# Xinglab/abPOA

Measured on AMD Instinct MI355X. Metric: read-sets/sec (consensus bit-exact) + DP Gcells/sec (roofline.dp_gcells_per_s), higher is better.
Workload: dtype int16

## Files before the change

### abpoa_amd/csrc/backtrack_dir.h

```cpp
#pragma once
#include "dp_common.h"
#include "dir_plane.h"
#include "rows_fast.h"
#include "backtrack.h"

namespace abpoa_hip {

constexpr int DBTR = 256;
constexpr int DIR_TRI_SLACK = 9;
constexpr int DIR_NA = -32768;
template <int R> struct __attribute__((aligned(16))) DirBtT { int2 rec[R]; int2 pd[R]; int32_t stg[R], rowA[R]; };
typedef DirBtT<DBTR> DirBt;

constexpr int SPEC_PM_ROWS = 256;
constexpr int SPEC_WK = 4;
__device__ __forceinline__ bool dir_walk_pair(const DevBatch &b, const AlnDesc &d) { return d.n_rows >= 768 && d.cigar_cap < 65536 && d.qlen < 65536 && b.ret_cigar; }
template <typename T, int GAP, int DBR = DBTR>
__device__ __forceinline__ void finish_alignment_dir(const DevBatch &b, const AlnDesc &d, AlnOut *out_rec, const TailState &ts, const int role = -1,
                                                     int *spec_ctl = nullptr, const int gen = 0) {
    constexpr int PN = Width<T>::PN, CW = FastFmt<T, GAP>::CW, DB = DirFmt<T, GAP>::DB, S = (int)sizeof(T);
    constexpr int ALIGN = 16 / DB;
    constexpr int DBL = DB == 2 ? 1 : 2;
    constexpr int NQ = DBR / 64;
    typedef DirBtT<DBR> DirBt;
    typedef typename std::conditional<GAP == 1, uint16_t, uint32_t>::type DW;
    typedef __attribute__((address_space(3))) unsigned char lds_byte_t;
    typedef __attribute__((address_space(3))) DW lds_dw_t;
    typedef int v2i_t __attribute__((ext_vector_type(2)));
    typedef __attribute__((address_space(3))) v2i_t lds_i2_t;
    typedef __attribute__((address_space(3))) int lds_i32_t;
    const int lane = threadIdx.x & 63;
    const int gn = d.n_rows, qlen = d.qlen;
    const int o1 = b.o1, o2 = b.o2;
    GLOBAL_AS const uint8_t *row_base = vgpr_ptr(b.row_base + d.row0);
    GLOBAL_AS const int32_t *row_node_id = vgpr_ptr(b.row_node_id + d.row0);
    GLOBAL_AS const uint32_t *row_pd = vgpr_ptr(b.row_pd + 2 * d.row0);
    GLOBAL_AS const int32_t *pred_off = vgpr_ptr(b.pred_off + d.poff0), *pred_row = vgpr_ptr(b.pred_row + d.pred0);
    GLOBAL_AS int32_t *g_bsn = vgpr_ptr(b.dp_beg_sn + d.row0), *g_esn = vgpr_ptr(b.dp_end_sn + d.row0);
    GLOBAL_AS int64_t *g_coff = vgpr_ptr(b.row_cell_off + d.row0);
    T *planes = (T *)(b.planes + d.plane_off);
    const unsigned char *arena = (const unsigned char *)planes;
    int status = ts.status, best_score = ts.best_score, best_i = ts.best_i, best_j = ts.best_j, bt_steps = 0;
    WG_SYNC();
    typedef __attribute__((address_space(3))) volatile int lds_vint_t;
    const bool spec_static = role >= 0 && dir_walk_pair(b, d), spec = spec_static && status == 0;
    auto start_row = [&](int r_) __attribute__((always_inline)) { return (int)(((long long)gn * (SPEC_WK - r_)) / SPEC_WK); };
    const int R_g = spec && role >= 1 ? start_row(role) : 0, R_lo = R_g - SPEC_PM_ROWS + 1;
    const int total_lds = b.lds.bt_off + b.lds.bt_bytes_tail;
    const int half_lds = spec_static ? ((total_lds - (SPEC_WK - 1) * SPEC_PM_ROWS * 4) / SPEC_WK) & ~15 : total_lds;
    int *pm_all = (int *)(lds_raw + b.lds.phase_off + SPEC_WK * half_lds);
    int *pm = pm_all + (role >= 1 ? role - 1 : 0) * SPEC_PM_ROWS;
    lds_vint_t *ctl = (lds_vint_t *)spec_ctl, *my = ctl + 8 * (role > 0 ? role : 0);
    auto helper_out = [&](int st_) __attribute__((always_inline)) { if (lane == 0) my[1] = st_; asm volatile("s_waitcnt lgkmcnt(0)" ::: "memory"); if (lane == 0) my[0] = gen; };
    if (role >= 1) {
        if (!spec) { if (spec_static) helper_out(-1); return; }
        const int c_g = __builtin_amdgcn_readfirstlane(gld_i32(vgpr_ptr(b.row_max_i + d.row0) + R_g));
        if (c_g < 1 || c_g > qlen) { helper_out(-1); return; }
        best_i = R_g; best_j = c_g;
    }

    const int cwr = takes_wide(b, d) ? (sizeof(T) == 2 ? (GAP == 2 ? 4 : 2) : 2) : CW;
    if (status == 0 && role < 1) {
        const int k0 = __builtin_amdgcn_readfirstlane(pred_off[gn - 1]), k1 = __builtin_amdgcn_readfirstlane(pred_off[gn]);
        for (int kb = k0; kb < k1; kb += 64) {
            const int k = kb + lane; const bool v = k < k1;
            int in_row = 0, end = 0, score = INT_MIN;
            if (v) {
                in_row = pred_row[k];
                const int pe = g_esn[in_row], pb = g_bsn[in_row];
                const int dpe = (pe + 1) * PN - 1; end = qlen > dpe ? dpe : qlen;
                score = (int)planes[g_coff[in_row] - (long long)(pe - pb + 1) * cwr * PN + (long long)(end - pb * PN) * cwr];
            }
            const int mx = wave_max_i32(score);
            if (mx > best_score) {
                const int first = __builtin_ctzll(__ballot(v && score == mx));
                best_score = mx; best_i = __builtin_amdgcn_readlane(in_row, first); best_j = __builtin_amdgcn_readlane(end, first);
            }
        }
    }

    int n_cigar = 0, node_s = 0, node_e = 0, query_s = 0, query_e = 0, n_aln = 0, n_match = 0;
    long long win_ticks = 0, walk_ticks = 0; int n_windows = 0, n_general = 0;
    long long dbg_why = 0, dbg_a = 0, dbg_b = 0;
    if (spec_static && role == 0) {
        for (int t = lane; t < (SPEC_WK - 1) * SPEC_PM_ROWS; t += 64) pm_all[t] = 0;
        asm volatile("s_waitcnt lgkmcnt(0)" ::: "memory");
        if (lane == 0) ctl[0] = gen;
    }
    if (status == 0 && b.ret_cigar && d.cigar_cap < gn + qlen + 2) status = ABPOA_HIP_EBACKTRACK;
    if (role >= 1 && status != 0) { helper_out(-1); return; }
    if (status == 0 && b.ret_cigar) {
        const int lds0 = b.lds.phase_off + (role >= 1 ? role * half_lds : 0);
        DirBt &B = *(DirBt *)(lds_raw + lds0);
        unsigned char *win = lds_raw + lds0 + (int)sizeof(DirBt);
        const int win_bytes = half_lds - (int)sizeof(DirBt);
        GLOBAL_AS uint64_t *cg = vgpr_ptr(b.cigar + d.cigar_off + (role >= 1 ? (long long)role * d.cigar_cap : 0));
        bool merged = false; int idx1 = 0, met = 0;
        int t_next = (role > 0 ? role : 0) + 1;
        int w_lo = 1, w_hi = 0, w_cref = 0; bool w_tri = false;
        unsigned nx_end = 0; bool nx_ok = false;
        auto load_window = [&](int hi, int jtop) __attribute__((always_inline)) -> int {
            const long long tw0 = (long long)__builtin_amdgcn_s_memtime(); ++n_windows;
            WG_SYNC();
            bool early = nx_ok && hi == w_lo - 1;
            const unsigned e_lo = nx_end > (unsigned)win_bytes ? nx_end - (unsigned)win_bytes : 0u;
            if (early) {
                const int n16 = (int)((nx_end - e_lo) >> 4);
                const int4 *src = (const int4 *)(arena + e_lo); int4 *dst = (int4 *)win;
                for (int i0 = 0; i0 < n16; i0 += 64) {
                    const int idx = i0 + lane;
                    if (idx < n16) __builtin_amdgcn_global_load_lds((const __attribute__((address_space(1))) void *)(src + idx), (__attribute__((address_space(3))) void *)(dst + i0), 16, 0, 0);
                }
            }
            const int cref = jtop - 4096;
            int bs[NQ], es[NQ]; long long co[NQ]; unsigned pdv[NQ], pdh[NQ];
#pragma unroll
            for (int q = 0; q < NQ; ++q) {
                const int r = hi - 64 * q - lane, rc = imax(r, 1);
                bs[q] = g_bsn[rc]; es[q] = g_esn[rc]; co[q] = g_coff[rc]; pdv[q] = row_pd[2 * rc]; pdh[q] = row_pd[2 * rc + 1];
            }
            int W[NQ], pc[NQ]; unsigned sa[NQ]; bool vq[NQ];
#pragma unroll
            for (int q = 0; q < NQ; ++q) { vq[q] = hi - 64 * q - lane >= 1; W[q] = (es[q] - bs[q] + 1) * PN; pc[q] = bs[q] * PN; sa[q] = (unsigned)(co[q] * S); }
            const unsigned end_hi = (unsigned)__builtin_amdgcn_readfirstlane((int)(sa[0] + (unsigned)(W[0] * DB)));
            int r_full = 0;
#pragma unroll
            for (int q = 0; q < NQ; ++q) r_full += __builtin_popcountll(__ballot(vq[q] && (early ? sa[q] >= e_lo : end_hi - sa[q] <= (unsigned)win_bytes)));
            if (early && r_full == 0) {
                asm volatile("s_waitcnt vmcnt(0)" ::: "memory");
                early = false; nx_ok = false;
#pragma unroll
                for (int q = 0; q < NQ; ++q) r_full += __builtin_popcountll(__ballot(vq[q] && end_hi - sa[q] <= (unsigned)win_bytes));
            }
            const bool narrow = early || r_full >= imin(16, hi);
            int sl[NQ], ns[NQ], off[NQ], R;
            unsigned s_lo = 0;
            if (narrow) {
                R = r_full;
                const int ql = (R - 1) >> 6, ll = (R - 1) & 63;
#pragma unroll
                for (int q = 0; q < NQ; ++q) if (q == ql) s_lo = (unsigned)__builtin_amdgcn_readlane((int)sa[q], ll);
                nx_end = s_lo;
                if (early) s_lo = e_lo;
#pragma unroll
                for (int q = 0; q < NQ; ++q) { sl[q] = pc[q]; ns[q] = W[q]; off[q] = (int)(sa[q] - s_lo); }
            } else {
                int run = 0; R = 0;
#pragma unroll
                for (int q = 0; q < NQ; ++q) {
                    const int tl = imax(pc[q], (jtop - 64 * q - lane - DIR_TRI_SLACK) & ~(ALIGN - 1)), th = imin(pc[q] + W[q], (jtop + ALIGN) & ~(ALIGN - 1));
                    sl[q] = tl; ns[q] = vq[q] ? imax(0, th - tl) : 0;
                    const int incl = run + wave_scan_add_i32(ns[q] * DB);
                    off[q] = incl - ns[q] * DB; run = __builtin_amdgcn_readlane(incl, 63);
                    R += __builtin_popcountll(__ballot(vq[q] && incl <= win_bytes));
                }
                if (R < 1) R = 1;
            }
            const int lo = hi - R + 1;
            nx_ok = narrow;
            if (narrow && early) {}
            else if (narrow) {
                const int n16 = (int)((end_hi - s_lo) >> 4);
                const int4 *src = (const int4 *)(arena + s_lo); int4 *dst = (int4 *)win;
                for (int i0 = 0; i0 < n16; i0 += 64) {
                    const int idx = i0 + lane;
                    if (idx < n16) __builtin_amdgcn_global_load_lds((const __attribute__((address_space(1))) void *)(src + idx), (__attribute__((address_space(3))) void *)(dst + i0), 16, 0, 0);
                }
            } else {
#pragma unroll
                for (int q = 0; q < NQ; ++q) {
                    const unsigned srcq = sa[q] + (unsigned)((sl[q] - pc[q]) * DB);
                    const int nrow = imin(64, R - 64 * q);
                    for (int u = 0; u < nrow; ++u) {
                        const int n_ = __builtin_amdgcn_readlane(ns[q], u) * DB / 16, ob = __builtin_amdgcn_readlane(off[q], u);
                        const unsigned so = (unsigned)__builtin_amdgcn_readlane((int)srcq, u);
                        const int4 *sp = (const int4 *)(arena + so); unsigned char *dp = win + ob;
                        for (int i0 = 0; i0 < n_; i0 += 64)
                            if (i0 + lane < n_) __builtin_amdgcn_global_load_lds((const __attribute__((address_space(1))) void *)(sp + i0 + lane),
                                    (__attribute__((address_space(3))) void *)(dp + i0 * 16), 16, 0, 0);
                    }
                }
            }
            int A[NQ];
#pragma unroll
            for (int q = 0; q < NQ; ++q) {
                A[q] = off[q] - ((sl[q] - cref) << DBL);
                const int li = hi - 64 * q - lane - lo;
                if (vq[q] && li >= 0) { B.rowA[li] = A[q]; B.pd[li] = make_int2((int)pdv[q], (int)pdh[q]); B.stg[li] = (sl[q] & 0x7fff) | ((sl[q] > pc[q] ? 1 : 0) << 15) | (ns[q] << 16); }
            }
            WG_SYNC();
#pragma unroll
            for (int q = 0; q < NQ; ++q) {
                const int r = hi - 64 * q - lane, li = r - lo;
                if (!(vq[q] && li >= 0)) continue;
                int pk[2];
#pragma unroll
                for (int k = 0; k < 2; ++k) {
                    const int dk = (int)((pdv[q] >> (8 * k)) & 0xffu), pr = r - dk; const bool in = dk != 255 && pr >= lo;
                    pk[k] = in ? (dk | (((B.rowA[pr - lo] >> 1) & 0xffff) << 8)) : 255;
                }
                B.rec[li] = make_int2(pk[0], pk[1]);
            }
            asm volatile("s_waitcnt vmcnt(0)" ::: "memory");
            WG_SYNC();
            w_lo = lo; w_hi = hi; w_cref = cref;
            win_ticks += (long long)__builtin_amdgcn_s_memtime() - tw0;
            w_tri = !narrow;
            return __builtin_amdgcn_readfirstlane(A[0]);
        };
        uint64_t last_word = 0; bool have_pending = false;
        auto store_word = [&](int idx, uint64_t wv) __attribute__((always_inline)) {
            GLOBAL_AS uint64_t *p_ = cg + idx;
            const int lo_ = (int)(wv & 0xffffffffull), hi_ = (int)(wv >> 32);
            asm volatile("global_store_dwordx2 %0, %1, off" :: "v"(p_), "v"(make_int2(lo_, hi_)) : "memory");
        };
        auto push = [&](int op, int len, int node_row, int query_id) __attribute__((always_inline)) {
            const uint64_t L = (uint64_t)(int64_t)len;
            if (n_cigar == 0 || op != ABPOA_HIP_CINS || op != (int)(last_word & 0xf)) {
                if (have_pending) store_word(n_cigar - 1, last_word);
                const uint64_t n_id = (uint64_t)(int64_t)node_row, q_id = (uint64_t)(int64_t)query_id;
                if (op == ABPOA_HIP_CMATCH) last_word = n_id << 34 | q_id << 4 | (uint64_t)op;
                else if (op == ABPOA_HIP_CINS) last_word = q_id << 34 | L << 4 | (uint64_t)op;
                else last_word = n_id << 34 | L << 4 | (uint64_t)op;
                have_pending = true; ++n_cigar;
            } else last_word += L << 4;
        };
        int runv = 0, run_n = 0, run_j = 0;
        auto flush_run = [&]() __attribute__((always_inline)) {
            if (run_n == 0) return;
            if (have_pending) { store_word(n_cigar - 1, last_word); have_pending = false; }
            if (spec) {
                const int row_ = lane < run_n ? runv : -1, col_ = run_j - lane;
                const int row_first = __builtin_amdgcn_readlane(runv, 0);
                while (t_next < SPEC_WK && row_first < start_row(t_next) - SPEC_PM_ROWS + 1) ++t_next;
                if (t_next < SPEC_WK) {
                    const int tl_ = row_ - (start_row(t_next) - SPEC_PM_ROWS + 1);
                    const bool in2 = row_ >= 0 && (unsigned)tl_ < (unsigned)SPEC_PM_ROWS;
                    const int e_ = in2 ? ((lds_vint_t *)(pm_all + (t_next - 1) * SPEC_PM_ROWS))[tl_] : 0;
                    const unsigned long long hit_ = __ballot(in2 && e_ != 0 && (e_ & 0xffff) == col_);
                    if (hit_) { const int f_ = __builtin_ctzll(hit_); idx1 = (int)((unsigned)__builtin_amdgcn_readlane(e_, f_) >> 16); met = t_next; run_n = f_; merged = true; if (run_n == 0) return;
                            }
                }
                if (role >= 1) { const int t_ = row_ - R_lo; if (lane < run_n && (unsigned)t_ < (unsigned)SPEC_PM_ROWS) pm[t_] = col_ | ((n_cigar + lane) << 16); }
            }
            if (lane < run_n) cg[n_cigar + lane] = (uint64_t)(unsigned)runv << 34 | (uint64_t)(unsigned)(run_j - 1 - lane) << 4 | (uint64_t)ABPOA_HIP_CMATCH;
// ... 210 lines not shown
```

### abpoa_amd/csrc/engine.cpp

```cpp
#include <hip/hip_runtime.h>
#include <stdio.h>
#include <stdlib.h>
#include <string.h>
#include <stdarg.h>
#include <limits.h>
#include <mutex>
#include <vector>
#include <algorithm>
#include "engine_options.h"
#include "batch_stream.h"
#include "dir_plane.h"

namespace abpoa_hip {

static char g_err[512] = ""; static std::mutex g_err_mu;
static thread_local char g_err_copy[512] = "";
static thread_local char tl_err[512] = "";
void set_err(const char *fmt, ...) {
    va_list ap; va_start(ap, fmt); vsnprintf(tl_err, sizeof(tl_err), fmt, ap); va_end(ap);
    std::lock_guard<std::mutex> lk(g_err_mu);
    memcpy(g_err, tl_err, sizeof(g_err));
}
const char *thread_last_error() { return tl_err; }
void clear_thread_error() { tl_err[0] = 0; }
#define HIP_TRY(expr, code)                                                                          \
    do { hipError_t e_ = (expr); if (e_ != hipSuccess) {                                             \
        set_err("%s failed: %s (%s:%d)", #expr, hipGetErrorString(e_), __FILE__, __LINE__); return code; } } while (0)

int Blob::reserve(size_t n) {
    if (n <= cap) return 0;
    size_t want = std::max(n, cap + cap / 2);
    want = (want + 0xFFFFF) & ~(size_t)0xFFFFF;
    release();
    if (hipMalloc((void **)&dev, want) != hipSuccess) { dev = nullptr; set_err("hipMalloc(%zu) failed", want); return ABPOA_HIP_ENOMEM; }
    if (mirrored && hipHostMalloc((void **)&host, want, hipHostMallocDefault) != hipSuccess) {
        host = nullptr; set_err("hipHostMalloc(%zu) failed", want); return ABPOA_HIP_ENOMEM; }
    cap = want; return 0;
}
void Blob::release() { if (dev) (void)hipFree(dev); if (host) (void)hipHostFree(host); dev = host = nullptr; cap = 0; }

struct Engine {
    bool ready = false; int device = -1;
    BatchStream flat;
    abpoa_hip_stats_t stats{};
    std::mutex mu, stats_mu;
};
static Engine g;
long long g_dbg[10] = {0};
long long g_dir_counts[2] = {0, 0};

int engine_device() { return g.ready ? g.device : -1; }
void add_global_stats(const StreamStats &s) {
    std::lock_guard<std::mutex> lk(g.stats_mu);
    g.stats.n_launches += s.n_launches; g.stats.n_alignments += s.n_alignments; g.stats.n_cells += s.n_cells;
    g.stats.algo_bytes += s.algo_bytes; g.stats.kernel_ms += s.kernel_ms; g.stats.h2d_ms += s.h2d_ms; g.stats.d2h_ms += s.d2h_ms; g.stats.tail_ms += s.tail_ms; g.stats.rounds_ms += s.rounds_ms;
    g.stats.rounds_launches += s.rounds_launches; g.stats.rounds_algo_bytes += s.rounds_algo_bytes;
}

static size_t align_up(size_t x, size_t a = 256) { return (x + a - 1) / a * a; }

int BatchStream::open(int device) {
    if (open_) return 0;
    HIP_TRY(hipSetDevice(device), ABPOA_HIP_ENODEV);
    HIP_TRY(hipStreamCreateWithFlags(&stream_, hipStreamNonBlocking), ABPOA_HIP_ENODEV);
    for (auto &e : ev_) HIP_TRY(hipEventCreate(&e), ABPOA_HIP_ENODEV);
    device_ = device; open_ = true; return 0;
}
void BatchStream::close() {
    if (!open_) return;
    (void)hipSetDevice(device_);
    (void)hipStreamSynchronize(stream_);
    in_.release(); out_.release(); planes_.release();
    for (auto &e : ev_) (void)hipEventDestroy(e);
    (void)hipStreamDestroy(stream_);
    open_ = false;
}

#ifdef ABPOA_HIP_WIDE_W3
constexpr int WIDE_PER_CU_MAX = 12, WIDE_RING_MIN = 2;
#else
constexpr int WIDE_PER_CU_MAX = 8, WIDE_RING_MIN = 4;
#endif
void make_lds_plan(const abpoa_hip_scoring_t *sc, int max_qlen, int max_bits, int64_t est_cols, int n_aln, LdsPlan *Lp) {
    LdsPlan &L = *Lp;
    const int P = sc->gap_mode == ABPOA_HIP_LINEAR_GAP ? 1 : (sc->gap_mode == ABPOA_HIP_AFFINE_GAP ? 3 : 5);
    const int cell = max_bits / 8, npr = P == 1 ? 1 : (P == 3 ? 2 : 3);
    const bool longq = max_qlen + 1 > 16384;
    L.q_off = 0; L.q_cap = max_qlen + 1 <= 32000 ? (int)align_up(max_qlen + 1, 16) : 0;
    L.mat_off = L.q_cap; L.mx_off = L.mat_off + (int)align_up(4 * sc->m * sc->m, 16);
    L.phase_off = L.mx_off + (int)align_up(4 * sc->m * (sc->m + 1), 16);
    L.ring_off = lds_fixed_bytes_dp(); L.ring_rows = 16; L.ring_cols = (int)align_up((size_t)est_cols, 64);
    while ((int64_t)L.ring_rows * npr * L.ring_cols * cell > 40 * 1024 && L.ring_rows > 4) L.ring_rows /= 2;
    if ((int64_t)L.ring_rows * npr * L.ring_cols * cell > 40 * 1024) L.ring_cols = 0;
    const int ring_bytes = L.ring_rows * npr * L.ring_cols * cell;
    L.bt_off = lds_fixed_bytes_bt();
    L.bt_bytes = std::max(std::max(8 * 1024, std::min(24 * 1024, (longq ? 62 : 38) * 1024 - L.phase_off - L.bt_off)), L.ring_off + ring_bytes - L.bt_off) & ~15;
    const int fw = P == 1 ? 1 : (max_bits == 16 ? (P == 3 ? 1 : 2) : (P == 3 ? 2 : 3));
    L.fr_off = 0; L.fr_rows = 16; L.fr_cols = fw ? std::max(128, (int)align_up((size_t)est_cols, 64)) : 0;
    const int fr_budget = (longq ? 62 : 36) * 1024 - L.phase_off;
    while (L.fr_cols && (int64_t)L.fr_rows * fw * (L.fr_cols + 4) * 4 + 64 > fr_budget && L.fr_rows > 4) L.fr_rows /= 2;
    if (L.fr_cols && (int64_t)L.fr_rows * fw * (L.fr_cols + 4) * 4 + 64 > fr_budget) L.fr_cols = 0;
    if (L.q_cap == 0 || est_cols > 1024) L.fr_cols = 0;
    { const char *nf_ = opt_env("ABPOA_HIP_NOFAST"); if (nf_ && atoi(nf_)) L.fr_cols = 0; }
    const int fr_bytes = L.fr_cols ? L.fr_rows * fw * (L.fr_cols + 4) * 4 + 64 : 0;
    L.total = L.phase_off + std::max(std::max(L.ring_off + ring_bytes, L.bt_off + L.bt_bytes), L.fr_off + fr_bytes);
    L.bt_bytes_tail = std::max(8 * 1024, std::min(28 * 1024, (longq ? 62 : 38) * 1024 - L.phase_off - L.bt_off)) & ~15;
    { const int per_cu = std::max(1, (n_aln + 255) / 256);
      if (per_cu < 4 && L.fr_cols > 128) L.bt_bytes_tail = std::max(L.bt_bytes_tail, std::min(56 * 1024, 160 * 1024 / per_cu - 2048 - L.phase_off - L.bt_off) & ~15); }
    if (n_aln > 4 * 256 && L.fr_cols && L.fr_cols <= 128) L.bt_bytes_tail = std::min(L.bt_bytes_tail, 12 * 1024);
    { const char *tb_ = opt_env("ABPOA_HIP_BT_BYTES"); if (tb_ && atoi(tb_) >= 4096 && atoi(tb_) <= 65536) L.bt_bytes_tail = atoi(tb_) & ~15; }
    L.total_rows = L.phase_off + L.fr_off + fr_bytes; L.total_tail = L.phase_off + L.bt_off + L.bt_bytes_tail;
    L.bt_wc = 0; { const char *wc_ = opt_env("ABPOA_HIP_BT_WC"); if (wc_ && atoi(wc_) >= 8 && atoi(wc_) <= 64) L.bt_wc = atoi(wc_) & ~7; }
    L.loc_rows = L.loc_cols = L.total_local = 0;
    if (sc->align_mode == ABPOA_HIP_LOCAL_MODE && sc->wb < 0 && P != 1 && L.q_cap && !(opt_env("ABPOA_HIP_NOFAST") && atoi(opt_env("ABPOA_HIP_NOFAST")))) {
        const int lw = P == 3 ? 1 : 2;
        L.loc_cols = 9 * 64; L.loc_rows = 16;
        while ((int64_t)L.loc_rows * lw * (L.loc_cols + 4) * 4 > 60 * 1024 - L.phase_off && L.loc_rows > 4) L.loc_rows /= 2;
        L.total_local = L.phase_off + L.fr_off + (int)align_up((size_t)L.loc_rows * lw * (L.loc_cols + 4) * 4, 16) + 256;
    }
    L.wide_nw = 0; L.wfr_rows = L.wfr_cols = L.wx_off = L.total_wide = 0; L.wide_w_lo = 1; L.wide_w_hi = 0; L.narrow_off = 0; L.w_mx_off = L.w_phase_off = 0;
    { const char *nw_ = opt_env("ABPOA_HIP_NOWIDE"), *mw_ = opt_env("ABPOA_HIP_TEAM");
      if (L.fr_cols && L.q_cap && !(nw_ && atoi(nw_))) {
          L.wide_nw = 1;
          if (mw_ && (atoi(mw_) == 1 || atoi(mw_) == 2 || atoi(mw_) == 4)) L.wide_nw = atoi(mw_);
          L.wfr_cols = (est_cols > WIDE_RING_COLS && !(opt_env("ABPOA_HIP_NOXL") && atoi(opt_env("ABPOA_HIP_NOXL")))) ? WIDE_RING_COLS_XL : WIDE_RING_COLS; L.wfr_rows = 16;
          if (sc->m > 16) L.wide_nw = 0;
          L.w_mx_off = (int)align_up((size_t)(max_qlen + 2) / 2, 16); L.w_phase_off = L.w_mx_off + (int)align_up(4 * sc->m * (sc->m + 1), 16);
          const int fww = (P == 5 && max_bits == 32) ? 2 : fw;
          if (P == 5 && (sc->gap_open1 + sc->gap_ext1 >= 65535 || sc->gap_open2 + sc->gap_ext2 >= 65535)) L.wide_nw = 0;
          L.wide_w_lo = 40; L.wide_w_hi = (L.wfr_cols - 2 * 8 - 1) / 2;
          { const char *lo_ = opt_env("ABPOA_HIP_WIDE_LO"); if (lo_ && atoi(lo_) > 0) L.wide_w_lo = atoi(lo_); }
          const char *rr_env_ = opt_env("ABPOA_HIP_RING_ROWS");
          if (rr_env_ && atoi(rr_env_) >= 4) L.wfr_rows = atoi(rr_env_) >= 16 ? 16 : (atoi(rr_env_) >= 8 ? 8 : 4); else rr_env_ = nullptr;
          const int budget = 120 * 1024 - L.w_phase_off - 512;
          while ((int64_t)L.wfr_rows * fww * (L.wfr_cols + 4) * 4 > budget && L.wfr_rows > 4) L.wfr_rows /= 2;
          const int extra_ = L.wide_nw > 1 ? 16 * 16 + 64 : 0;
          auto per_cu_ = [&](int rows_) { return std::min<int64_t>(WIDE_PER_CU_MAX, 128 / ((L.w_phase_off + (int64_t)rows_ * fww * (L.wfr_cols + 4) * 4 + extra_ + 1279) / 1280)); };
          if (!(rr_env_)) {
              const int top_ = L.wfr_rows; int best_ = top_;
              for (int r_ = top_; r_ >= WIDE_RING_MIN; r_ /= 2) {
                  if (per_cu_(r_) > per_cu_(best_)) best_ = r_;
                  if (per_cu_(r_) * 256 >= std::min(n_aln, WIDE_PER_CU_MAX * 256)) { best_ = r_; break; }
              }
              L.wfr_rows = best_;
          }
          L.wx_off = L.fr_off + (int)align_up((size_t)L.wfr_rows * fww * (L.wfr_cols + 4) * 4, 16);
          L.total_wide = L.w_phase_off + L.wx_off + extra_;
          if (P == 1) L.wide_nw = 0;
      } }
}

int BatchStream::prepare(const abpoa_hip_scoring_t *sc, int n, const BatchShape *sh, unsigned flags) {
    if (!open_) { set_err("stream not open"); return ABPOA_HIP_ENODEV; }
    HIP_TRY(hipSetDevice(device_), ABPOA_HIP_ENODEV);
    sc_ = *sc; mat_.assign(sc->mat, sc->mat + sc->m * sc->m); sc_.mat = mat_.data();
    flags_ = flags; n_ = n;
    P_ = sc->gap_mode == ABPOA_HIP_LINEAR_GAP ? 1 : (sc->gap_mode == ABPOA_HIP_AFFINE_GAP ? 3 : 5);
    const bool banded = sc->wb >= 0;
    desc_.resize(n); recs_.resize(n); full_cells_.resize(n); est_cells_.resize(n); dir_full_cells_.resize(n); dir_est_cells_.resize(n); trace_arena_.clear();
    rows_tot_ = preds_tot_ = outs_tot_ = q_tot_ = cig_tot_ = 0;
    for (int i = 0; i < n; ++i) {
        AlnDesc &d = desc_[i];
        d.n_rows = sh[i].n_rows; d.qlen = sh[i].qlen;
        d.bits = abpoa_hip_score_bits(sc, d.n_rows, d.qlen, &d.inf_min);
        d.w = sc->wb < 0 ? d.qlen : sc->wb + (int)(sc->wf * d.qlen);
        d.cigar_cap = d.n_rows + d.qlen + 8;
        d.query_off = q_tot_; d.row0 = rows_tot_; d.poff0 = rows_tot_ + i; d.pred0 = preds_tot_; d.out0 = outs_tot_; d.cigar_off = cig_tot_;
        q_tot_ += d.qlen; rows_tot_ += d.n_rows; preds_tot_ += sh[i].n_pred; outs_tot_ += sh[i].n_out; cig_tot_ += d.cigar_cap;
        const int pn = d.bits == 16 ? 16 : 8;
        const int64_t width = (int64_t)((d.qlen + pn) / pn) * pn;
        const int pv = sc->gap_mode == ABPOA_HIP_LINEAR_GAP ? 2 : (sc->gap_mode == ABPOA_HIP_AFFINE_GAP ? 4 : 8);
        full_cells_[i] = width * pv * d.n_rows;
        int64_t est = banded ? std::min<int64_t>(width, 2LL * d.w + 3 * pn + 32) : width;
        { const char *pct_ = opt_env("ABPOA_HIP_ARENA_PCT"); if (pct_ && atoi(pct_) > 0 && atoi(pct_) < 100) est = std::max<int64_t>(pn, est * atoi(pct_) / 100); }
        d.plane_cap = std::min<int64_t>(full_cells_[i], width * pv + est * pv * (d.n_rows - 1));
        est_cells_[i] = d.plane_cap;
        const int64_t dbc = (sc->gap_mode == ABPOA_HIP_AFFINE_GAP ? 2 : 4) * 8 / d.bits + 1;
        dir_full_cells_[i] = width * (pv + dbc) * d.n_rows + 64;
        dir_est_cells_[i] = std::min<int64_t>(dir_full_cells_[i], width * (pv + dbc) + (est * dbc + est * pv / 4 + 2 * pn) * (d.n_rows - 1));
    }
    size_t o = 0;
    auto take = [&](size_t bytes) { size_t at = o; o = align_up(o + bytes); return at; };
    o_desc_ = take(sizeof(AlnDesc) * n); o_mat_ = take(sizeof(int32_t) * sc->m * sc->m); o_query_ = take(q_tot_ + 1);
    o_base_ = take(rows_tot_); o_sdist_ = take(rows_tot_); o_pd_ = take(8 * rows_tot_); o_nid_ = take(4 * rows_tot_); o_rem_ = take(4 * rows_tot_); o_act_ = take(rows_tot_);
    o_poff_ = take(4 * (rows_tot_ + n)); o_pred_ = take(4 * (preds_tot_ + 1)); o_ooff_ = take(4 * (rows_tot_ + n)); o_out_ = take(4 * (outs_tot_ + 1) + 4 * 512);
    in_bytes_ = o;
    o = 0;
    o_rec_ = take(sizeof(AlnOut) * n); o_cig_ = take(8 * cig_tot_); o_left_ = take(4 * rows_tot_); o_right_ = take(4 * rows_tot_);
    o_bsn_ = take(4 * rows_tot_); o_esn_ = take(4 * rows_tot_); o_coff_ = take(8 * rows_tot_); o_rmi_ = take(4 * rows_tot_);
    out_bytes_ = o;
    int rc;
    if ((rc = in_.reserve(in_bytes_)) || (rc = out_.reserve(out_bytes_))) return rc;
    memcpy(in_.host + o_mat_, sc->mat, sizeof(int32_t) * sc->m * sc->m);
    memset(in_.host + o_act_, 1, rows_tot_);
    return 0;
}

ProblemSlots BatchStream::slots(int i) const {
    const AlnDesc &d = desc_[i]; uint8_t *hi = in_.host, *ho = out_.host; ProblemSlots s;
    s.query = hi + o_query_ + d.query_off; s.row_base = hi + o_base_ + d.row0;
    s.row_node_id = (int32_t *)(hi + o_nid_) + d.row0; s.row_remain = (int32_t *)(hi + o_rem_) + d.row0; s.row_active = hi + o_act_ + d.row0;
    s.pred_off = (int32_t *)(hi + o_poff_) + d.poff0; s.pred_row = (int32_t *)(hi + o_pred_) + d.pred0;
    s.out_off = (int32_t *)(hi + o_ooff_) + d.poff0; s.out_row = (int32_t *)(hi + o_out_) + d.out0;
    s.left = (int32_t *)(ho + o_left_) + d.row0; s.right = (int32_t *)(ho + o_right_) + d.row0;
    return s;
}
const uint64_t *BatchStream::cigar(int i) const { return (const uint64_t *)(out_.host + o_cig_) + desc_[i].cigar_off; }
const int32_t *BatchStream::left(int i) const { return (const int32_t *)(out_.host + o_left_) + desc_[i].row0; }
const int32_t *BatchStream::right(int i) const { return (const int32_t *)(out_.host + o_right_) + desc_[i].row0; }

int BatchStream::run() {
    HIP_TRY(hipSetDevice(device_), ABPOA_HIP_ENODEV);
    const abpoa_hip_scoring_t *sc = &sc_;
    const bool banded = sc->wb >= 0, trace = flags_ & BS_TRACE, fresh = flags_ & BS_FRESH_BAND;
    const int P = P_, n = n_;
    uint8_t *hi = in_.host, *ho = out_.host, *di = in_.dev, *dout = out_.dev;
    std::vector<int> todo(n); for (int i = 0; i < n; ++i) todo[i] = i;
    const size_t lr_words = (o_right_ - o_left_) / 4 + rows_tot_;
    std::vector<int32_t> saved_lr;
    bool first_pass = true; int rc;
    std::vector<AlnDesc> pass;
    const bool dirtrace = trace && opt_env("ABPOA_HIP_DIRTRACE") && atoi(opt_env("ABPOA_HIP_DIRTRACE"));
    bool dir = (!trace || dirtrace) && banded && sc->align_mode == ABPOA_HIP_GLOBAL_MODE && dir_plane_usable(sc->gap_mode, sc->gap_open1, sc->gap_ext1, sc->gap_open2, sc->gap_ext2) &&
               !(opt_env("ABPOA_HIP_NODIR") && atoi(opt_env("ABPOA_HIP_NODIR"))) && !(opt_env("ABPOA_HIP_TEAM") && atoi(opt_env("ABPOA_HIP_TEAM")) > 1);
    for (int i = 0; i < n; ++i) {
        AlnDesc &d = desc_[i]; bool ok = banded || (sc->align_mode == ABPOA_HIP_LOCAL_MODE && sc->wb < 0);
        if (ok && memchr(hi + o_act_ + d.row0, 0, (size_t)d.n_rows)) ok = false;
        if (ok && banded && !fresh) {
            const int32_t *l = (const int32_t *)(ho + o_left_) + d.row0, *r = (const int32_t *)(ho + o_right_) + d.row0;
            for (int k = 0; k < d.n_rows && ok; ++k) ok = l[k] == d.n_rows && r[k] == 0;
        }
        d.flags = ok ? ALN_FAST_OK : 0; d.pad0 = 0;
    }
    if (dir) {
        for (int i = 0; i < n; ++i) {
            AlnDesc &d = desc_[i];
            if (!(d.flags & ALN_FAST_OK)) continue;
            const int32_t *po = (const int32_t *)(hi + o_poff_) + d.poff0, *pr = (const int32_t *)(hi + o_pred_) + d.pred0; uint8_t *sd = hi + o_sdist_ + d.row0;
            uint32_t *pdw = (uint32_t *)(hi + o_pd_) + 2 * d.row0;
            memset(sd, 0, (size_t)d.n_rows);
            bool ok = true;
            for (int r = 0; r < d.n_rows && ok; ++r) {
                const int np_ = po[r + 1] - po[r];
                if (np_ > DIR_K_MAX && r < d.n_rows - 1) ok = false;
                uint64_t pdv = ~0ull;
                for (int k = po[r]; k < po[r + 1]; ++k) {
                    const int p_ = pr[k], dist = r == d.n_rows - 1 ? 255 : std::min(255, r - p_); if (dist > sd[p_]) sd[p_] = (uint8_t)dist;
                    const int t = k - po[r]; if (t < 8 && r - p_ <= 254) pdv = (pdv & ~(0xffull << (8 * t))) | ((uint64_t)(r - p_) << (8 * t));
                }
                (void)np_;
                pdw[2 * r] = (uint32_t)pdv; pdw[2 * r + 1] = (uint32_t)(pdv >> 32);
            }
            if (!ok) d.flags = 0;
        }
    }
    while (!todo.empty()) {
        int64_t plane_bytes = 0;
        pass.resize(todo.size());
        for (size_t t = 0; t < todo.size(); ++t) pass[t] = desc_[todo[t]];
        DevBatch b; memset(&b, 0, sizeof(b));
        b.n = (int)pass.size(); b.m = sc->m;
        {
            int max_qlen = 0, max_bits = 16; int64_t est_cols = 0;
            for (const AlnDesc &d : pass) {
// ... 302 lines not shown
```

### abpoa_amd/csrc/engine.h

```cpp
#pragma once
#include <stdint.h>
#include <hip/hip_runtime.h>
#include "../../include/abpoa_hip.h"

namespace abpoa_hip {

struct AlnDesc {
    int32_t n_rows, qlen;
    int32_t bits;
    int32_t inf_min;
    int32_t w;
    int32_t cigar_cap;
    int32_t flags;
    int32_t pad0;
    int64_t query_off;
    int64_t row0;
    int64_t poff0;
    int64_t pred0;
    int64_t out0;
    int64_t plane_off;
    int64_t plane_cap;
    int64_t cigar_off;
};

struct AlnOut {
    int32_t status;
    int32_t best_score, best_row, best_col;
    int32_t node_s, node_e, query_s, query_e;
    int32_t n_aln_bases, n_matched_bases;
    int32_t n_cigar;
    int32_t pad;
    int64_t n_cells;
    int64_t cells_used;
    int64_t clk_dp, clk_bt;
    int32_t n_rows_done, n_bt_steps;
    int64_t seg[6];
};

#define ALN_FAST_OK 1
#define ALN_SKIP 2
#define WIDE_RING_COLS 448
#define WIDE_RING_COLS_XL 704
#define ABPOA_HIP_STATUS_OVERFLOW 1
#define ABPOA_HIP_STATUS_NEED_SCORES 2

struct LdsPlan {
    int32_t q_off, q_cap;
    int32_t mat_off;
    int32_t phase_off;
    int32_t ring_rows, ring_cols;
    int32_t ring_off;
    int32_t bt_off, bt_bytes;
    int32_t bt_bytes_tail;
    int32_t bt_wc;
    int32_t fr_off, fr_rows, fr_cols;
    int32_t wfr_rows, wfr_cols, wx_off, wide_nw;
    int32_t wide_w_lo, wide_w_hi;
    int32_t narrow_off;
    int32_t total_wide;
    int32_t w_mx_off, w_phase_off;
    int32_t loc_rows, loc_cols, total_local;
    int32_t mx_off;
    int32_t total;
    int32_t total_rows, total_tail;
};

struct DevBatch {
    int32_t n;
    int32_t m;
    int32_t o1, e1, o2, e2;
    int32_t align_mode, gap_mode, wb, zdrop, ret_cigar, rev_cigar;
    int32_t want_trace;
    int32_t dbg;
    int32_t fresh_band;
    int32_t want_lr;
    int32_t bits_mask;
    int32_t dir_mode;
    int32_t pad1;
    LdsPlan lds;
    const int32_t *mat;
    const AlnDesc *aln;
    AlnOut *out;
    const uint8_t *query;
    const uint8_t *row_base;
    const int32_t *row_node_id;
    const int32_t *row_remain;
    const uint8_t *row_active;
    const uint8_t *row_sdist;
    const uint32_t *row_pd;
    const int32_t *pred_off;
    const int32_t *pred_row;
    const int32_t *out_off;
    const int32_t *out_row;
    int32_t *left, *right;
    int32_t *dp_beg_sn, *dp_end_sn;
    int64_t *row_cell_off;
    int32_t *row_max_i;
    uint8_t *planes;
    uint64_t *cigar;
};

constexpr int LINEAR_FAST_W = 40;
__host__ __device__ inline bool fast_global_job(int gap_mode, int align_mode, int wb, int e1) {
    if (wb < 0) return false;
    if (gap_mode == ABPOA_HIP_LINEAR_GAP && e1 < 1) return false;
    return align_mode == ABPOA_HIP_GLOBAL_MODE || align_mode == ABPOA_HIP_EXTEND_MODE;
}
__host__ __device__ inline bool fast_global_aln(int gap_mode, int w, int pad0) { return gap_mode != ABPOA_HIP_LINEAR_GAP || w + (pad0 >> 1) < LINEAR_FAST_W; }

int lds_fixed_bytes_dp();
int lds_fixed_bytes_bt();

hipError_t launch_dp(const DevBatch &b, int n_fast, hipStream_t stream, hipEvent_t after_rows);
hipError_t launch_dp_fast(const DevBatch &b, hipStream_t stream, hipEvent_t after_rows);
hipError_t launch_dp_general(const DevBatch &b, hipStream_t stream);

}
```

### abpoa_amd/csrc/engine_options.cpp

```cpp
#include "engine_options.h"
#include <atomic>
#include <cstdlib>
#include <cstring>
#include <mutex>
#include <string>

namespace abpoa_hip {
namespace {

struct Row { const char *name, *help; };
const Row kTable[] = {
    {"ABPOA_GPU_DEVICES", "P  device ordinals abpoa_hip_msa_batch spreads its batches over: all | 0,1,... (default: the device of abpoa_hip_init)"},
    {"ABPOA_GPU_BATCHES_PER_DEVICE", "P  batches dealt per device queue [2]"},
    {"ABPOA_HIP_STRICT", "P  1: a call that would hand any read-set to the host driver fails with ABPOA_HIP_ESTRICT"},
    {"ABPOA_HIP_VERBOSE", "P  per-pass timings, residency and fallback reasons on stderr"},
    {"ABPOA_HIP_HOSTGRAPH", "T  1: the host driver for every job"},
    {"ABPOA_HIP_NO_DEVICE_STRAND", "T  1: -s jobs on the host driver"},
    {"ABPOA_HIP_NO_DEVICE_LOCAL", "T  1: local-mode jobs on the host driver"},
    {"ABPOA_HIP_NO_DEVICE_GENERAL", "T  1: general-kernel jobs on the host driver"},
    {"ABPOA_HIP_DEVICE_GENERAL", "T  1: the general kernel for every device-resident job"},
    {"ABPOA_HIP_LOCKSTEP", "T  1: one launch per phase and round also where the all-rounds kernel would run"},
    {"ABPOA_HIP_NODIR", "T  1: score-record arenas instead of direction words"},
    {"ABPOA_HIP_DIR_WIDE", "T  1 / 0: direction words for wide-band alignments always / never (default: by residency and memory)"},
    {"ABPOA_HIP_NOFAST", "T  1: no fast row loops (general kernel)"},
    {"ABPOA_HIP_NOWIDE", "T  1: no wide row loop"},
    {"ABPOA_HIP_NOXL", "T  1: no long-read form of the wide row loop"},
    {"ABPOA_HIP_TEAM", "T  1 | 2 | 4 wavefronts per wide-band alignment"},
    {"ABPOA_HIP_LOCAL_TEAM", "T  1 / 0: the four-wavefront local row loop always / never"},
    {"ABPOA_HIP_WIDE_LO", "T  smallest band half-width that takes the wide loop [40]"},
    {"ABPOA_HIP_RING_ROWS", "T  depth of the wide loop's score ring (4 | 8 | 16)"},
    {"ABPOA_HIP_EXTRA_ROUTE_MIN", "T  ragged sets with fewer extra columns keep the narrow loop"},
    {"ABPOA_HIP_NO_RAGGED_SPLIT", "T  1: read-sets with ragged read ends stay in the batch of the uniform ones (no all-rounds kernel for such a job)"},
    {"ABPOA_HIP_RAGGED_CONCURRENT", "T  1: the ragged batch of a mixed job runs on a second queue of the device beside the uniform batch (measured: see LOG.md)"},
    {"ABPOA_HIP_PASS_SETS", "T  read-sets per pass of the device-resident driver"},
    {"ABPOA_HIP_FIRST_PASS", "T  start the node-slot ladder at pass 1 / 2 / 3 (profiling runs of one step)"},
    {"ABPOA_HIP_NO_PASS_HINT", "T  1: always start the ladder at 3x"},
    {"ABPOA_HIP_GROUPS", "T  read-set groups of the host driver"},
    {"ABPOA_HIP_ARENA_PCT", "T  arena estimate in percent (overflow-retry tests)"},
    {"ABPOA_HIP_BT_BYTES", "T  LDS window of the tail kernel in bytes"},
    {"ABPOA_HIP_BT_WC", "T  columns per row of the tail's column-slice windows"},
    {"ABPOA_HIP_ORDER_LDS", "T  0: the row-order walk with global tables"},
    {"ABPOA_HIP_ORDER_CAP", "T  node capacity of the row-order walk's LDS tables"},
    {"ABPOA_HIP_DBG", "D  bit mask handed to the kernels (DevBatch.dbg: 64 no fast loops, 128 keep counters, 1024 one wavefront per backtrack, 2048 the compiler's tight loop, ...)"},
    {"ABPOA_HIP_DEVSYNC", "D  1: compare device graph / row order / MSA with the host's after every read"},
    {"ABPOA_HIP_DEVICE_AUDIT", "D  1: every pool of a device queue must sit on that queue's device"},
    {"ABPOA_HIP_CIGAR_DIGEST", "D  1: fold every graph cigar into a per-set digest on the device"},
    {"ABPOA_HIP_DIRTRACE", "D  1: keep direction words and scores (word-level tests)"},
    {"ABPOA_HIP_IMBAL", "D  1: per-round mean / slowest alignment"},
    {"ABPOA_HIP_WIDE_COUNTERS", "D  path census of the wide loop (diagnostic build)"},
    {"ABPOA_HIP_ROW_CENSUS", "D  row census of the narrow loop (diagnostic build)"},
    {"ABPOA_HIP_ORDER_PROF", "D  in-kernel clock of the row-order walk (diagnostic build)"},
};
constexpr int N = (int)(sizeof(kTable) / sizeof(kTable[0]));

struct Snap { bool set[N]; std::string val[N]; };
std::mutex g_mu;
bool g_over_on[N]; std::string g_over[N];
std::atomic<const Snap *> g_snap{nullptr};

int find(const char *name) { for (int i = 0; i < N; ++i) if (strcmp(kTable[i].name, name) == 0) return i; return -1; }

}

void refresh_options() {
    std::lock_guard<std::mutex> lk(g_mu);
    Snap s;
    for (int i = 0; i < N; ++i) {
        const char *e = g_over_on[i] ? g_over[i].c_str() : getenv(kTable[i].name);
        s.set[i] = e != nullptr; s.val[i] = e ? e : "";
    }
    const Snap *cur = g_snap.load(std::memory_order_acquire);
    bool same = cur != nullptr;
    for (int i = 0; same && i < N; ++i) same = cur->set[i] == s.set[i] && cur->val[i] == s.val[i];
    if (!same) g_snap.store(new Snap(s), std::memory_order_release);
}

const char *opt_env(const char *name) {
    const Snap *cur = g_snap.load(std::memory_order_acquire);
    if (!cur) { refresh_options(); cur = g_snap.load(std::memory_order_acquire); }
    const int i = find(name);
    return (i >= 0 && cur->set[i]) ? cur->val[i].c_str() : nullptr;
}

int set_option(const char *name, const char *value) {
    const int i = name ? find(name) : -1;
    if (i < 0) return -1;
    { std::lock_guard<std::mutex> lk(g_mu); g_over_on[i] = value != nullptr; g_over[i] = value ? value : ""; }
    refresh_options();
    return 0;
}

int list_options(const char **names, const char **help, int cap) {
    for (int i = 0; i < N && i < cap; ++i) { if (names) names[i] = kTable[i].name; if (help) help[i] = kTable[i].help; }
    return N;
}

}
```

### abpoa_amd/csrc/fast_tail.h

```cpp
#pragma once
#include "rows_fast.h"
#include "rows_local.h"
#include "backtrack.h"
#include "backtrack_dir.h"

namespace abpoa_hip {

template <typename T, int GAP, bool DIR = false>
__device__ __forceinline__ void align_fast_tail(const DevBatch &b, const AlnDesc &d, AlnOut *out_rec, const int role = -1, int *spec_ctl = nullptr, const int gen = 0) {
    const int lane = threadIdx.x & 63;
    if (role >= 1) {
        if (!(DIR && takes_dir(b, d) && dir_walk_pair(b, d))) return;
        typedef __attribute__((address_space(3))) volatile int lds_vint_t;
        while (((lds_vint_t *)spec_ctl)[0] != gen) __builtin_amdgcn_s_sleep(4);
    }
    uint8_t *s_query = lds_raw + b.lds.q_off;
    int32_t *s_mat = (int32_t *)(lds_raw + b.lds.mat_off);
    const bool dir_a = DIR && takes_dir(b, d);
    if (!dir_a) { GLOBAL_AS const int32_t *g_mat = vgpr_ptr(b.mat); for (int i = lane; i < b.m * b.m; i += 64) s_mat[i] = g_mat[i]; }
    if (!dir_a) { GLOBAL_AS const uint8_t *g_query = vgpr_ptr(b.query + d.query_off); for (int i = lane; i < d.qlen; i += 64) s_query[i] = g_query[i]; }
    TailState ts;
    ts.status = out_rec->status; ts.n_cells = out_rec->n_cells; ts.cursor = out_rec->cells_used; ts.rows_done = out_rec->n_rows_done;
    ts.best_score = d.inf_min; ts.best_i = 0; ts.best_j = 0;
    if (b.align_mode == ABPOA_HIP_LOCAL_MODE || b.align_mode == ABPOA_HIP_EXTEND_MODE) { ts.best_score = out_rec->best_score; ts.best_i = out_rec->best_row; ts.best_j = out_rec->best_col; }
    for (int i_ = 0; i_ < 6; ++i_) ts.seg[i_] = out_rec->seg[i_];
    ts.clk1 = (long long)__builtin_amdgcn_s_memtime(); ts.clk0 = ts.clk1 - out_rec->clk_dp;
    WG_SYNC();
    if constexpr (DIR) {
        if (!takes_dir(b, d)) finish_alignment<T, GAP, FastFmt<T, GAP>::CW>(b, d, out_rec, ts);
        else if (role >= 0 && dir_walk_pair(b, d)) finish_alignment_dir<T, GAP, 64>(b, d, out_rec, ts, role, spec_ctl, gen);
        else if (role <= 0) finish_alignment_dir<T, GAP>(b, d, out_rec, ts);
    }
    else finish_alignment<T, GAP, FastFmt<T, GAP>::CW>(b, d, out_rec, ts);
}

}
```

### abpoa_amd/csrc/msa_device.cpp

```cpp
#include <algorithm>
#include <atomic>
#include <chrono>
#include <limits.h>
#include <mutex>
#include <stdio.h>
#include <stdlib.h>
#include <string.h>
#include <thread>
#include <vector>
#include <hip/hip_runtime.h>
#include "engine_options.h"
#include "batch_stream.h"
#include "msa_device.h"
#include "poa_device.h"
#include "poa_graph.h"
#include "dir_plane.h"
#include "msa_batch.h"
#include "msa_device_debug.h"

namespace abpoa_hip {

namespace {
#define HIP_OK(expr, code) do { hipError_t e_ = (expr); if (e_ != hipSuccess) { \
        set_err("%s failed: %s (%s:%d)", #expr, hipGetErrorString(e_), __FILE__, __LINE__); return code; } } while (0)
// ... 82 lines not shown
    const bool fast = fast_global_job(sc->gap_mode, sc->align_mode, sc->wb, sc->gap_ext1) || (sc->gap_mode != ABPOA_HIP_LINEAR_GAP && sc->align_mode == ABPOA_HIP_LOCAL_MODE);
    if (!fast && opt_env("ABPOA_HIP_NO_DEVICE_GENERAL") && atoi(opt_env("ABPOA_HIP_NO_DEVICE_GENERAL"))) return false;
    return true;
}

int msa_device_resident_sets(const abpoa_hip_scoring_t *sc, int n_sets, const abpoa_hip_readset_t *sets) {
    int max_qlen = 0; for (int s = 0; s < n_sets; ++s) for (int r = 0; r < sets[s].n_reads; ++r) max_qlen = std::max(max_qlen, sets[s].lens[r]);
    if (max_qlen <= 0) return 0;
    const int w_max = sc->wb + (int)(sc->wf * (float)max_qlen);
    LdsPlan pl; int32_t inf_d; const int mb = abpoa_hip_score_bits(sc, 3 * max_qlen + 1024, max_qlen, &inf_d); const int pn_ = mb == 16 ? 16 : 8;
    make_lds_plan(sc, max_qlen, mb, std::min<int64_t>((int64_t)((max_qlen + pn_) / pn_) * pn_, 2LL * w_max + 3 * pn_ + 32), n_sets, &pl);
    if (pl.wide_nw != 1 || !(w_max >= pl.wide_w_lo && w_max <= pl.wide_w_hi) || pl.total_wide <= 0) return 0;
    int dev = 0, cus = 256; if (hipGetDevice(&dev) == hipSuccess) { hipDeviceProp_t pr;
            if (hipGetDeviceProperties(&pr, dev) == hipSuccess && pr.multiProcessorCount > 0) cus = pr.multiProcessorCount; }
#ifdef ABPOA_HIP_WIDE_W3
    const int per_cu = std::max(1, std::min(12, 128 / ((pl.total_wide + 1279) / 1280)));
#else
    const int per_cu = std::max(1, std::min(8, 128 / ((pl.total_wide + 1279) / 1280)));
#endif
    return per_cu * cus;
}

static int run_msa_device_body(const abpoa_hip_scoring_t *sc_in, int n_sets, const abpoa_hip_readset_t *sets, abpoa_hip_msa_t *out, int n_threads,
                               std::vector<int> *fallback, DeviceRunStats *stats, double node_factor, unsigned flags, int device, int slot, bool force_general, bool *want_general,
                               std::vector<int> *fallback_reason) {
    abpoa_hip_scoring_t sc_norm = *sc_in; const bool local = sc_in->align_mode == ABPOA_HIP_LOCAL_MODE, extend = sc_in->align_mode == ABPOA_HIP_EXTEND_MODE;
    if (local) sc_norm.wb = -1;
    const abpoa_hip_scoring_t *sc = &sc_norm;
    const bool amb = flags & ABPOA_HIP_AMB_STRAND;
    const bool want_msa = flags & ABPOA_HIP_OUT_MSA, want_cons = (flags & ABPOA_HIP_OUT_CONS) || !want_msa;
    if (slot < 0 || slot >= MSA_DEVICE_SLOTS) { set_err("bad device slot %d", slot); return ABPOA_HIP_EINVAL; }
    std::lock_guard<std::mutex> lk(g_cache_mu[slot]);
    Cache &C = g_cache[slot];
    if (device < 0) device = engine_device();
    if (device < 0) { set_err("engine not initialised"); return ABPOA_HIP_ENODEV; }
    HIP_OK(hipSetDevice(device), ABPOA_HIP_ENODEV);
    t_queue_device = device;
    if (C.device != device) {
        if (C.device >= 0) {
            (void)hipSetDevice(C.device);
            for (Arena *a : {&C.in, &C.graph, &C.rows, &C.planes, &C.out, &C.msa}) { if (a->dev) (void)hipFree(a->dev);
                    if (a->host) (void)hipHostFree(a->host); *a = Arena(); }
            if (C.stream) (void)hipStreamDestroy(C.stream); if (C.copy_stream) (void)hipStreamDestroy(C.copy_stream);
            if (C.ev_copy) (void)hipEventDestroy(C.ev_copy);
            for (hipEvent_t e : C.ev) (void)hipEventDestroy(e);
            C = Cache();
            HIP_OK(hipSetDevice(device), ABPOA_HIP_ENODEV);
        }
        if (!C.stream) HIP_OK(hipStreamCreateWithFlags(&C.stream, hipStreamNonBlocking), ABPOA_HIP_ENODEV);
        C.device = device;
    }
    fallback->clear();
    if (stats) memset(stats, 0, sizeof(*stats));
    const double t_begin = now_s();
    const int CW = sc->gap_mode == ABPOA_HIP_LINEAR_GAP ? 2 : (sc->gap_mode == ABPOA_HIP_AFFINE_GAP ? 4 : 8);
    const bool unbanded = sc->wb < 0;
    int max_reads = 0, max_qlen = 0; int64_t tot_reads = 0, tot_bases = 0, max_cap0 = 0;
    for (int s = 0; s < n_sets; ++s) {
        max_reads = std::max(max_reads, sets[s].n_reads); tot_reads += sets[s].n_reads;
        int64_t sum = 0; int mx = 0;
        for (int r = 0; r < sets[s].n_reads; ++r) { max_qlen = std::max(max_qlen, sets[s].lens[r]); mx = std::max(mx, sets[s].lens[r]); sum += sets[s].lens[r];
                }
        tot_bases += sum; max_cap0 = std::max(max_cap0, std::min<int64_t>(2 + sum, 2 + (int64_t)(node_factor * mx) + 1024));
    }
    bool general;
    {   LdsPlan pl; int32_t inf_d; const int mb = abpoa_hip_score_bits(sc, (int)max_cap0, max_qlen, &inf_d); const int pn_ = mb == 16 ? 16 : 8;
        const int64_t width_ = (int64_t)((max_qlen + pn_) / pn_) * pn_, w_ = sc->wb + (int)(sc->wf * (float)max_qlen);
        make_lds_plan(sc, max_qlen, mb, (local || unbanded) ? width_ : std::min<int64_t>(width_, 2LL * w_ + 3 * pn_ + 32), n_sets, &pl);
        bool fast_global = fast_global_job(sc->gap_mode, sc->align_mode, sc->wb, sc->gap_ext1) && pl.fr_cols > 0 && max_qlen <= pl.q_cap;
        if (fast_global && sc->gap_mode == ABPOA_HIP_LINEAR_GAP) {
            if (w_ >= LINEAR_FAST_W) fast_global = false;
            for (int s = 0; s < n_sets && fast_global; ++s) if (msa_device_set_is_ragged(sets[s])) fast_global = false;
        }
        const bool fast_local = local && sc->gap_mode != ABPOA_HIP_LINEAR_GAP && mb == 16 && pl.loc_cols > 0 && (max_qlen / 16 + 1) * 16 <= pl.loc_cols
                && max_qlen <= pl.q_cap;
        general = !(fast_global || fast_local);
        if (opt_env("ABPOA_HIP_DEVICE_GENERAL") && atoi(opt_env("ABPOA_HIP_DEVICE_GENERAL"))) general = true;
        if (force_general) general = true;
    }
    const bool roomy = node_factor >= 4096.0;
    const int in_cap = roomy ? std::max((int)POA_IN_CAP, std::min(250, max_reads + 1)) : POA_IN_CAP, out_cap = roomy ? std::max((int)POA_OUT_CAP, std::min(250, max_reads + 1)) : POA_OUT_CAP;
    const bool dir = !local && !extend && !general && !amb && in_cap <= POA_IN_CAP && dir_plane_usable(sc->gap_mode, sc->gap_open1, sc->gap_ext1, sc->gap_open2,
            sc->gap_ext2) && !(opt_env("ABPOA_HIP_NODIR") && atoi(opt_env("ABPOA_HIP_NODIR"))) &&
                     !(opt_env("ABPOA_HIP_TEAM") && atoi(opt_env("ABPOA_HIP_TEAM")) > 1);
    const int DB = sc->gap_mode == ABPOA_HIP_AFFINE_GAP ? 2 : 4;

    std::vector<PoaSet> ps(n_sets);
    int64_t node_tot = 0, pred_tot = 0, cig_tot = 0, scr_tot = 0, plane_tot = 0, read_i = 0, cons_tot = 0, term_tot = 0; int max_node_cap = 0;
    const int w_max = sc->wb + (int)(sc->wf * (float)max_qlen);
    const int aln_cap = std::max(1, sc->m - 1), rid_words = want_msa ? std::max(1, (max_reads + 63) / 64) : 0;
    auto est_cols = [&](int64_t width, int w, int pn) { return (local || unbanded) ? width : std::min<int64_t>(width, 2LL * w + 3 * pn + 32); };
    int wide_lo = 1, wide_hi = 0, wide_ring_rows = 16;
    { LdsPlan pl; int32_t inf_d; const int mb = abpoa_hip_score_bits(sc, 3 * max_qlen + 1024, max_qlen, &inf_d); const int pn_ = mb == 16 ? 16 : 8;
      make_lds_plan(sc, max_qlen, mb, est_cols((int64_t)((max_qlen + pn_) / pn_) * pn_, w_max, pn_), n_sets, &pl);
      if (pl.wide_nw >= 1 && !local && !general) { wide_lo = pl.wide_w_lo; wide_hi = pl.wide_w_hi; wide_ring_rows = pl.wfr_rows; } }
    std::vector<int> extra(n_sets, 0), route(n_sets, 0); int max_extra = 0, weff_lo = INT_MAX, weff_hi = 0;
    const int route_min = opt_env("ABPOA_HIP_EXTRA_ROUTE_MIN") ? atoi(opt_env("ABPOA_HIP_EXTRA_ROUTE_MIN")) : 0;
    if (!local && !general && sc->wb >= 0) for (int s = 0; s < n_sets; ++s) {
        int mx = 0, mn = INT_MAX; for (int r = 0; r < sets[s].n_reads; ++r) { mx = std::max(mx, sets[s].lens[r]); mn = std::min(mn, sets[s].lens[r]); }
        if (sets[s].n_reads < 2) continue;
        const int spread = mx - mn, tol = std::max(64, mx / 8);
        extra[s] = spread > tol ? std::min((spread + 15) & ~15, 2048) : 0;
        max_extra = std::max(max_extra, extra[s]);
        route[s] = extra[s] >= route_min ? extra[s] : 0;
        weff_lo = std::min(weff_lo, sc->wb + (int)(sc->wf * (float)mn) + route[s] / 2);
        weff_hi = std::max(weff_hi, sc->wb + (int)(sc->wf * (float)mx) + route[s] / 2);
    }
    if (weff_hi == 0) { weff_lo = 0; }
    const bool lin_fast = !general && !local && !extend && sc->gap_mode == ABPOA_HIP_LINEAR_GAP && !amb;
    const bool rounds_possible = (dir || lin_fast) && max_reads > 2 && !(w_max >= wide_lo && wide_hi >= wide_lo) && max_extra == 0;
    bool dir_wide = false, any_wide_set = false;
    { const char *e_ = opt_env("ABPOA_HIP_DIR_WIDE"); if (dir && e_ && atoi(e_) > 0) dir_wide = true; }
    const bool dir_wide_auto = dir && !opt_env("ABPOA_HIP_DIR_WIDE");
    if (dir_wide_auto && wide_ring_rows <= 4 && wide_hi >= wide_lo) dir_wide = true;
    for (int s = 0; s < n_sets; ++s) {
        PoaSet &S = ps[s]; memset(&S, 0, sizeof(S));
        int64_t sum = 0; int mx = 0;
        for (int r = 0; r < sets[s].n_reads; ++r) { sum += sets[s].lens[r]; mx = std::max(mx, sets[s].lens[r]); }
        const int64_t cap = std::min<int64_t>(2 + sum, 2 + (int64_t)((node_factor + (extra[s] > 0 ? 1.0 : 0.0)) * mx) + 1024);
        S.n_reads = sets[s].n_reads; S.node_cap = (int)cap; S.pred_cap = (int)(4 * cap);
        S.read0 = read_i; read_i += sets[s].n_reads;
        S.term0 = term_tot; term_tot += sets[s].n_reads + 2;
        S.node0 = node_tot; node_tot += cap + 1;
        S.pred0 = pred_tot; pred_tot += S.pred_cap;
        S.cigar_cap = (int)(cap + mx + 8); S.cigar_off = cig_tot; cig_tot += ((rounds_possible && S.cigar_cap < 65536) ? 4 : 1) * (int64_t)S.cigar_cap;
        S.scratch0 = scr_tot; scr_tot += 3LL * max_qlen + 4 * cap + 8;
        S.cons_cap = (int)std::min<int64_t>(cap, 2LL * mx + 64); S.cons0 = cons_tot; cons_tot += S.cons_cap;
        const int w = sc->wb + (int)(sc->wf * (float)mx) + route[s] / 2;
        S.band_extra = route[s];
        max_node_cap = std::max(max_node_cap, (int)cap);
        any_wide_set |= (w >= wide_lo && w <= wide_hi);
    }
    auto size_arenas = [&](bool dw) {
        plane_tot = 0;
        for (int s = 0; s < n_sets; ++s) {
            PoaSet &S = ps[s]; int mx = 0; for (int r = 0; r < sets[s].n_reads; ++r) mx = std::max(mx, sets[s].lens[r]);
            const int64_t cap = S.node_cap;
            int32_t inf_dummy; const int bits = abpoa_hip_score_bits(sc, (int)cap, mx, &inf_dummy); const int pn = bits == 16 ? 16 : 8;
            const int64_t width = (int64_t)((mx + pn) / pn) * pn;
            const int w = sc->wb + (int)(sc->wf * (float)mx);
            int64_t est = std::min<int64_t>(width, est_cols(width, w, pn) + extra[s]);
            int64_t sum_len = 0; for (int r = 0; r < sets[s].n_reads; ++r) sum_len += sets[s].lens[r];
            const bool slots_fixed = 2 + sum_len <= 2 + (int64_t)(3.0 * mx) + 1024;
            if (node_factor > 3.0 && (roomy || slots_fixed)) {
                const double cellb = dir ? (double)(DB + 8) : (double)CW * (bits / 8);
                int64_t e2 = roomy ? width : std::min<int64_t>(width, (int64_t)((double)est * node_factor / 3.0));
                if (roomy && (double)e2 * (double)cap * cellb > 1e9) e2 = std::min<int64_t>(width, est * 4);
                est = std::max(est, e2);
            }
            const bool wide_s = !local && w + route[s] / 2 >= wide_lo && w + route[s] / 2 <= wide_hi;
            const bool dir_s = dir && (dw || !wide_s);
            const int64_t rec_div = (wide_s && wide_ring_rows <= 4) ? 2 : 4;
            const int64_t recb = wide_s ? ((bits == 16 && CW == 4) ? 4 : 8) : CW * (bits / 8);
            const int64_t bytes = local ? (int64_t)up((size_t)((width * cap + 64) * CW * (bits / 8) + 64 * 8 * 4))
                                : dir_s ? (int64_t)up((size_t)(width * (DB + recb) + (est * DB + est * recb / rec_div + 32) * (cap - 1) + 64 * 8 * 4))
                                      : (int64_t)up((size_t)((width + est * (cap - 1)) * CW * (bits / 8) + 64 * 8 * 4));
            S.plane_off = plane_tot; S.plane_cap = bytes - 64 * 8 * 4; plane_tot += bytes;
        }
    };
    size_arenas(dir_wide);
    Layout L; size_t o = 0;
    auto take = [&](size_t bytes) { size_t at = o; o = up(o + bytes); return at; };
    L.o_sets = take(sizeof(PoaSet) * n_sets); L.o_roff = take(8 * (tot_reads + 1)); L.o_rlen = take(4 * (tot_reads + 1)); L.o_mat = take(4 * sc->m * sc->m);
    L.o_rargs = take(poa_rounds_args_bytes()); L.o_msaoff_h = take(want_msa ? 8 * (size_t)n_sets : 0);
    bool any_w = false; for (int s = 0; s < n_sets && !any_w; ++s) any_w = sets[s].weights != nullptr;
    L.o_wts = take(any_w ? 4 * (size_t)(tot_bases + 64) : 0);
    L.o_reads = take(tot_bases + 64); L.in_bytes = o;
    L.o_rc = take(amb ? tot_bases + 64 : 0); L.o_wrc = take(amb && any_w ? 4 * (size_t)(tot_bases + 64) : 0); L.in_dev_bytes = o;
    o = 0;
    L.o_state = take(sizeof(PoaState) * n_sets);
    L.o_cnode = take(4 * cons_tot); L.o_ccov = take(4 * cons_tot); L.o_cbase = take(cons_tot); L.o_isrc = take(amb ? (size_t)tot_reads : 0);
    const size_t dl_bytes = o;
    L.o_order0 = take(4 * node_tot); L.o_order1 = take(4 * node_tot); L.o_base = take(node_tot); L.o_nout = take(node_tot);
    L.o_out = take(4 * node_tot * POA_HOT); L.o_outw = take(4 * node_tot * POA_HOT); L.o_nread = take(4 * node_tot);
    L.o_outx = take(4 * node_tot * (size_t)(out_cap - POA_HOT)); L.o_outwx = take(4 * node_tot * (size_t)(out_cap - POA_HOT));
    L.o_inx = take(4 * node_tot * (size_t)(in_cap - POA_HOT));
    L.o_nin = take(node_tot); L.o_naln = take(node_tot); L.o_in = take(4 * node_tot * POA_HOT); L.o_aln = take(4 * node_tot * (size_t)aln_cap);
    L.o_row = take(4 * node_tot);
    L.o_rid = take(8 * node_tot * (size_t)out_cap * (size_t)rid_words); L.o_mrank = take(want_msa ? 4 * node_tot : 0);
    L.o_msaoff = take(want_msa ? 8 * (size_t)n_sets : 0);
    L.o_tout = take(4 * term_tot); L.o_toutw = take(4 * term_tot); L.o_tin = take(4 * term_tot);
    L.graph_bytes = o;
    o = 0;
    L.o_ticket = take(4 * POA_CU_TICKETS);
    L.o_aln_desc = take(sizeof(AlnDesc) * n_sets); L.o_out_rec = take(sizeof(AlnOut) * n_sets);
    L.o_rbase = take(node_tot); L.o_rsd = take(node_tot); L.o_rpd = take(8 * node_tot); L.o_rnid = take(4 * node_tot); L.o_rrem = take(4 * node_tot);
    L.o_poff = take(4 * node_tot); L.o_pred = take(4 * (pred_tot + 1));
    L.o_bsn = take(4 * node_tot); L.o_esn = take(4 * node_tot); L.o_coff = take(8 * node_tot); L.o_rmi = take(4 * node_tot);
    L.o_cigar = take(8 * cig_tot); L.o_scratch = take(4 * scr_tot);
    const bool gen_io = general || amb;
    L.o_ooff = take(gen_io ? 4 * node_tot : 0); L.o_orow = take(gen_io ? 4 * (pred_tot + 1) : 0); L.o_left = take(gen_io ? 4 * node_tot : 0);
    L.o_right = take(gen_io ? 4 * node_tot : 0); L.o_act = take(gen_io ? node_tot : 0);
    L.o_outfwd = take(amb ? sizeof(AlnOut) * n_sets : 0); L.o_cigfwd = take(amb ? 8 * cig_tot : 0); L.o_retry = take(amb ? (size_t)n_sets : 0);
    L.rows_bytes = o;

    {
        size_t free_b = 0, total_b = 0; (void)hipMemGetInfo(&free_b, &total_b);
        const size_t want[4] = {L.in_dev_bytes, L.graph_bytes, L.rows_bytes, (size_t)plane_tot}, have[4] = {C.in.dev_cap, C.graph.dev_cap, C.rows.dev_cap,
                C.planes.dev_cap};
        size_t need = 0, given_back = 0;
        for (int i = 0; i < 4; ++i) if (want[i] > have[i]) { need += want[i]; given_back += have[i]; }
        if (need > free_b + given_back && dir_wide_auto && any_wide_set && !dir_wide) {
            dir_wide = true; size_arenas(true);
            need = 0; given_back = 0;
            const size_t want2[4] = {L.in_dev_bytes, L.graph_bytes, L.rows_bytes, (size_t)plane_tot};
            for (int i = 0; i < 4; ++i) if (want2[i] > have[i]) { need += want2[i]; given_back += have[i]; }
            if (opt_env("ABPOA_HIP_VERBOSE")) fprintf(stderr,
                    "[abpoa-hip] device %d: %d sets: score-record arenas do not fit, direction words for the wide-band sets " "too (arenas %.1f GB)\n", device,
                    n_sets, plane_tot / 1e9);
        }
        if (need > free_b + given_back) {
            if (opt_env("ABPOA_HIP_VERBOSE")) fprintf(stderr,
                    "[abpoa-hip] device %d: %d sets need %.1f GB in growing buffers (arenas %.1f GB), %.1f GB free + %.1f " "GB given back: splitting\n",
                    device, n_sets, need / 1e9, plane_tot / 1e9, free_b / 1e9, given_back / 1e9);
            set_err("device-resident job needs %zu more bytes, %zu free", need, free_b + given_back); return ABPOA_HIP_ENOMEM;
        }
    }
    int rc;
    if ((rc = C.in.need_dev(L.in_dev_bytes)) || (rc = C.in.need_host(L.in_bytes)) || (rc = C.graph.need_dev(L.graph_bytes)) || (rc =
            C.graph.need_host(dl_bytes)) ||
        (rc = C.rows.need_dev(L.rows_bytes)) || (rc = C.planes.need_dev((size_t)plane_tot))) return rc;
    const int n_ev = 4 * max_reads + 8;
    while ((int)C.ev.size() < n_ev) { hipEvent_t e; HIP_OK(hipEventCreate(&e), ABPOA_HIP_ENODEV); C.ev.push_back(e); }

    uint8_t *hi = C.in.host;
    memcpy(hi + L.o_sets, ps.data(), sizeof(PoaSet) * n_sets);
    int64_t *roff = (int64_t *)(hi + L.o_roff); int32_t *rlen = (int32_t *)(hi + L.o_rlen); uint8_t *rd = hi + L.o_reads;
    int64_t split_at = 0;
    {
        int64_t at = 0;
        for (int k = 0; k < max_reads; ++k) {
            if (k == 2) split_at = at;
            for (int s = 0; s < n_sets; ++s) if (k < sets[s].n_reads) { const int64_t ri = ps[s].read0 + k; roff[ri] = at; rlen[ri] = sets[s].lens[k];
                    at += sets[s].lens[k]; }
        }
        if (max_reads <= 2) split_at = at;
        roff[tot_reads] = at;
    }
    auto stage_reads = [&](int k_lo, int k_hi) {
        parallel_ranges(std::min(n_threads, 16), n_sets, [&](int lo, int hi_) {
            for (int s = lo; s < hi_; ++s) { const int64_t r0 = ps[s].read0; const int ke = std::min(k_hi, sets[s].n_reads);
                    for (int r = k_lo; r < ke; ++r) memcpy(rd + roff[r0 + r], sets[s].seqs[r], sets[s].lens[r]); }
        });
    };
    stage_reads(0, 2);
    if (any_w) {
        int32_t *wd = (int32_t *)(hi + L.o_wts);
        parallel_ranges(std::min(n_threads, 16), n_sets, [&](int lo, int hi_) {
            for (int s = lo; s < hi_; ++s) for (int r = 0; r < sets[s].n_reads; ++r) {
                int32_t *dst = wd + roff[ps[s].read0 + r]; const int32_t *src = sets[s].weights ? sets[s].weights[r] : nullptr;
                if (src) memcpy(dst, src, 4 * (size_t)sets[s].lens[r]); else for (int j = 0; j < sets[s].lens[r]; ++j) dst[j] = 1;
            }
        });
    }
    memcpy(hi + L.o_mat, sc->mat, 4 * sc->m * sc->m);
    hipStream_t st = C.stream;
    if (!C.copy_stream) { HIP_OK(hipStreamCreateWithFlags(&C.copy_stream, hipStreamNonBlocking), ABPOA_HIP_ENODEV);
            HIP_OK(hipEventCreateWithFlags(&C.ev_copy, hipEventDisableTiming), ABPOA_HIP_ENODEV); }
    HIP_OK(hipMemcpyAsync(C.in.dev, hi, L.o_reads + (size_t)split_at, hipMemcpyHostToDevice, st), ABPOA_HIP_ELAUNCH);
    bool rest_up = split_at >= roff[tot_reads];

    uint8_t *di = C.in.dev, *dg = C.graph.dev, *dr = C.rows.dev;
    PoaDev p; memset(&p, 0, sizeof(p));
    p.n_sets = n_sets; p.m = sc->m; p.max_mat = sc->max_mat; p.min_mis = sc->min_mis; p.o1 = sc->gap_open1; p.e1 = sc->gap_ext1; p.o2 = sc->gap_open2;
    p.e2 = sc->gap_ext2;
    p.wb = sc->wb; p.wf = sc->wf; p.gap_mode = sc->gap_mode; p.max_qlen = max_qlen;
    p.last_pass = node_factor >= 6.0 ? 1 : 0;
    p.in_cap = in_cap; p.out_cap = out_cap;
    p.dig_on = cigar_digest_on() ? 1 : 0;
    p.aln_cap = aln_cap; p.rid_words = rid_words; p.order_mode = (local || extend) ? 1 : 0; p.banded = (sc->wb >= 0 || sc->zdrop > 0) ? 1 : 0;
    p.general = general ? 1 : 0; p.msa_rows = 0; p.msa_cons = (want_msa && want_cons) ? 1 : 0;
    p.order_lds = (p.order_mode || want_msa) ? std::min(((max_node_cap + 3) & ~3), 6000) : 0;
    p.order_ecap = p.order_mode ? std::max(1024, std::min(65535, (40 * 1024 - 128 - 13 * p.order_lds) / 2)) : 0;
    { const char *e_ = opt_env("ABPOA_HIP_ORDER_LDS"); if (e_ && !atoi(e_)) p.order_ecap = 0; }
    { const char *e_ = opt_env("ABPOA_HIP_ORDER_CAP"); if (e_ && atoi(e_) >= 0) p.order_lds = std::min(p.order_lds, atoi(e_) & ~3); }
    p.pad = max_node_cap <= 8000 ? ((max_node_cap + 3) & ~3) : 0;
    p.sets = (const PoaSet *)(di + L.o_sets); p.state = (PoaState *)(dg + L.o_state);
    p.read_off = (const int64_t *)(di + L.o_roff); p.read_len = (const int32_t *)(di + L.o_rlen); p.reads = di + L.o_reads;
    p.wts = any_w ? (const int32_t *)(di + L.o_wts) : nullptr;
    p.nd_base = dg + L.o_base; p.nd_nin = dg + L.o_nin; p.nd_nout = dg + L.o_nout; p.nd_naln = dg + L.o_naln;
    p.nd_in = (int32_t *)(dg + L.o_in); p.nd_out = (int32_t *)(dg + L.o_out); p.nd_outw = (int32_t *)(dg + L.o_outw); p.nd_aln = (int32_t *)(dg + L.o_aln);
    p.nd_inx = (int32_t *)(dg + L.o_inx); p.nd_outx = (int32_t *)(dg + L.o_outx); p.nd_outwx = (int32_t *)(dg + L.o_outwx);
    p.nd_nread = (int32_t *)(dg + L.o_nread); p.nd_row = (int32_t *)(dg + L.o_row);
    p.t_out = (int32_t *)(dg + L.o_tout); p.t_outw = (int32_t *)(dg + L.o_toutw); p.t_in = (int32_t *)(dg + L.o_tin);
    p.nd_rid = (uint64_t *)(dg + L.o_rid); p.msa_rank = (int32_t *)(dg + L.o_mrank); p.msa_off = (const int64_t *)(dg + L.o_msaoff); p.msa_out = nullptr;
    p.row_node[0] = (int32_t *)(dg + L.o_order0); p.row_node[1] = (int32_t *)(dg + L.o_order1);
    p.scratch = (int32_t *)(dr + L.o_scratch);
    p.aln = (AlnDesc *)(dr + L.o_aln_desc); p.out = (AlnOut *)(dr + L.o_out_rec);
    p.row_base = dr + L.o_rbase; p.row_sdist = dr + L.o_rsd; p.row_pd = (uint32_t *)(dr + L.o_rpd); p.row_node_id = (int32_t *)(dr + L.o_rnid);
    p.row_remain = (int32_t *)(dr + L.o_rrem);
    p.pred_off = (int32_t *)(dr + L.o_poff); p.pred_row = (int32_t *)(dr + L.o_pred); p.cigar = (uint64_t *)(dr + L.o_cigar);
    p.out_off = gen_io ? (int32_t *)(dr + L.o_ooff) : nullptr; p.out_row = gen_io ? (int32_t *)(dr + L.o_orow) : nullptr;
    if (amb) {
        p.reads_rc = di + L.o_rc; p.wts_rc = any_w ? (int32_t *)(di + L.o_wrc) : nullptr; p.is_rc = dg + L.o_isrc; p.retry = dr + L.o_retry;
        p.out_fwd = (AlnOut *)(dr + L.o_outfwd); p.cigar_fwd = (uint64_t *)(dr + L.o_cigfwd);
    }
    p.cons_node = (int32_t *)(dg + L.o_cnode); p.cons_cov = (int32_t *)(dg + L.o_ccov); p.cons_base = dg + L.o_cbase;

    DevBatch b; memset(&b, 0, sizeof(b));
    b.n = n_sets; b.m = sc->m;
    {
        int32_t inf_dummy; const int max_bits = abpoa_hip_score_bits(sc, max_node_cap, max_qlen, &inf_dummy); const int pn = max_bits == 16 ? 16 : 8;
        const int64_t width = (int64_t)((max_qlen + pn) / pn) * pn;
        const int64_t est_plain = est_cols(width, w_max, pn), est_ragged = std::min<int64_t>(std::max<int64_t>(est_plain, std::min<int64_t>(1024, width)),
                est_plain + max_extra);
        make_lds_plan(sc, max_qlen, max_bits, est_ragged, n_sets, &b.lds);
        if (max_extra > 0 && b.lds.fr_cols == 0) make_lds_plan(sc, max_qlen, max_bits, est_plain, n_sets, &b.lds);
        if (general) { b.lds.wide_nw = 0; b.lds.fr_cols = 0; b.lds.loc_cols = 0; }
        else if (local) {
            b.lds.wide_nw = 0;
            if (max_bits != 16 || b.lds.loc_cols <= 0 || (max_qlen / 16 + 1) * 16 > b.lds.loc_cols || max_qlen > b.lds.q_cap) {
                    set_err("local alignment outside the device row loop's range"); return ABPOA_HIP_EINVAL; }
        }
        int min_qlen = max_qlen;
        for (int s = 0; s < n_sets; ++s) for (int r = 1; r < sets[s].n_reads; ++r) min_qlen = std::min(min_qlen, sets[s].lens[r]);
        const int min_bits = abpoa_hip_score_bits(sc, 3, min_qlen, &inf_dummy);
        b.bits_mask = (min_bits == 16 ? 1 : 0) | (max_bits == 32 ? 2 : 0);
        const int w_min = std::min(sc->wb + (int)(sc->wf * (float)min_qlen), max_extra ? weff_lo : INT_MAX), w_top = std::max(w_max, weff_hi);
        const bool mixed = max_extra > 0;
        if (!mixed && (w_top < b.lds.wide_w_lo || w_min > b.lds.wide_w_hi)) b.lds.wide_nw = 0;
        b.lds.narrow_off = (!mixed && b.lds.wide_nw >= 1 && w_min >= b.lds.wide_w_lo && w_top <= b.lds.wide_w_hi) ? 1 : 0;
    }
    if (!local && !general && (b.lds.fr_cols == 0 || max_qlen > b.lds.q_cap)) { *want_general = true; set_err("band too wide for the fast row loop"); return ABPOA_HIP_EINVAL; }
    b.o1 = sc->gap_open1; b.e1 = sc->gap_ext1; b.o2 = sc->gap_open2; b.e2 = sc->gap_ext2;
    b.align_mode = sc->align_mode; b.gap_mode = sc->gap_mode; b.wb = sc->wb; b.zdrop = sc->zdrop; b.ret_cigar = 1; b.rev_cigar = 0;
    b.want_trace = 0; b.fresh_band = 1; b.want_lr = 0; b.dbg = 0;
    { const char *dbg_ = opt_env("ABPOA_HIP_DBG"); if (dbg_) b.dbg = atoi(dbg_); }
    b.mat = (const int32_t *)(di + L.o_mat); b.aln = p.aln; b.out = p.out;
    b.dir_mode = (dir && b.lds.wide_nw <= 1) ? (dir_wide ? 2 : 1) : 0; b.row_sdist = p.row_sdist; b.row_pd = p.row_pd;
    b.query = p.reads; b.row_base = p.row_base; b.row_node_id = p.row_node_id; b.row_remain = p.row_remain; b.row_active = p.row_base;
    b.pred_off = p.pred_off; b.pred_row = p.pred_row; b.out_off = p.pred_off; b.out_row = p.pred_row;
    b.left = p.scratch; b.right = p.scratch;
    if (gen_io) {
        b.out_off = p.out_off; b.out_row = p.out_row; b.left = (int32_t *)(dr + L.o_left); b.right = (int32_t *)(dr + L.o_right); b.row_active = dr + L.o_act;
        HIP_OK(hipMemsetAsync(dr + L.o_act, 1, (size_t)node_tot, st), ABPOA_HIP_ELAUNCH);
    }
    b.dp_beg_sn = (int32_t *)(dr + L.o_bsn); b.dp_end_sn = (int32_t *)(dr + L.o_esn); b.row_cell_off = (int64_t *)(dr + L.o_coff);
    b.row_max_i = (int32_t *)(dr + L.o_rmi);
    b.planes = C.planes.dev; b.cigar = p.cigar;
    DevBatch b_rc = b;
    if (amb) {
        HIP_OK(hipMemsetAsync(dg + L.o_isrc, 0, (size_t)tot_reads, st), ABPOA_HIP_ELAUNCH);
        b.want_lr = (sc->wb >= 0 && !general) ? 1 : 0;
        b_rc = b; b_rc.want_lr = 0; b_rc.fresh_band = sc->wb >= 0 ? 0 : 1;
    }

    const bool dbg_sync = opt_env("ABPOA_HIP_DEVSYNC") && atoi(opt_env("ABPOA_HIP_DEVSYNC"));
    bool use_rounds = !local && rounds_possible && !dbg_sync && b.lds.wide_nw == 0 && !(b.dbg & 64) && max_reads > 2 && !(opt_env("ABPOA_HIP_LOCKSTEP")
            && atoi(opt_env("ABPOA_HIP_LOCKSTEP")));
    DevBatch b_r = b; size_t rounds_lds = 0;
    if (use_rounds) {
        auto dyn_of = [&](const DevBatch &x) { return std::max<size_t>(std::max<size_t>((size_t)x.lds.total_rows, (size_t)x.lds.total_tail),
                std::max<size_t>((size_t)5 * (size_t)(p.pad > 0 ? p.pad : 0), (size_t)16 * 256)); };
        rounds_lds = dyn_of(b_r);
        int st_lds = 0; int nb = poa_rounds_residency(sc->gap_mode, rounds_lds, &st_lds);
        if (nb < 4 && n_sets > nb * 256) {
            const int budget = 160 * 1024 / 4 - st_lds - 512, excess = (int)rounds_lds - budget;
            if (excess > 0 && (size_t)b_r.lds.total_tail == rounds_lds && b_r.lds.bt_bytes_tail - ((excess + 15) & ~15) >= 8 * 1024) {
                b_r.lds.bt_bytes_tail -= (excess + 15) & ~15; b_r.lds.total_tail -= (excess + 15) & ~15;
                rounds_lds = dyn_of(b_r); nb = poa_rounds_residency(sc->gap_mode, rounds_lds, &st_lds);
            }
        }
        int n_cu = 256; { hipDeviceProp_t pr; if (hipGetDeviceProperties(&pr, device) == hipSuccess && pr.multiProcessorCount > 0) n_cu =
                pr.multiProcessorCount; }
        if (nb < 1 || n_sets > nb * n_cu) use_rounds = false;
        if (opt_env("ABPOA_HIP_VERBOSE")) fprintf(stderr,
                "[abpoa-hip] all-rounds kernel: %s, %zu B dynamic + %d B static LDS per workgroup, %d workgroups per CU, " "backtrack window %d B\n",
                use_rounds ? "on" : "off", rounds_lds, st_lds, nb, b_r.lds.bt_bytes_tail);
    }

    DeviceDebug dbg(&p, &ps, sets, n_sets, sc->m, aln_cap, max_reads, want_msa, amb, st);
    auto stage = [&](const char *what, int k) { return dbg.stage(what, k); };
    const double t_queue = now_s();
    HIP_OK(hipEventRecord(C.ev[0], st), ABPOA_HIP_ELAUNCH);
    if (stage("upload", 0)) return ABPOA_HIP_ELAUNCH;
    HIP_OK(launch_poa_init(p, st), ABPOA_HIP_ELAUNCH);
    if (stage("init", 0)) return ABPOA_HIP_ELAUNCH;
    dbg.graph_check(0);
    HIP_OK(hipEventRecord(C.ev[1], st), ABPOA_HIP_ELAUNCH);
    for (int k = 1; k < max_reads; ++k) {
        if (k == 2 && !rest_up) {
            stage_reads(2, max_reads);
            HIP_OK(hipMemcpyAsync(C.in.dev + L.o_reads + (size_t)split_at, hi + L.o_reads + (size_t)split_at, (size_t)(roff[tot_reads] - split_at),
                    hipMemcpyHostToDevice, C.copy_stream), ABPOA_HIP_ELAUNCH);
            HIP_OK(hipEventRecord(C.ev_copy, C.copy_stream), ABPOA_HIP_ELAUNCH);
            HIP_OK(hipStreamWaitEvent(st, C.ev_copy, 0), ABPOA_HIP_ELAUNCH);
            rest_up = true;
        }
        if (use_rounds && k == 2) {
            HIP_OK(hipEventRecord(C.ev[2], st), ABPOA_HIP_ELAUNCH);
            HIP_OK(launch_poa_rounds(p, b_r, (int32_t *)(dr + L.o_ticket), C.in.host + L.o_rargs, slot, 2, rounds_lds, st), ABPOA_HIP_ELAUNCH);
            HIP_OK(hipEventRecord(C.ev[3], st), ABPOA_HIP_ELAUNCH);
            break;
        }
        p.round = k;
        hipEvent_t *e = C.ev.data() + 4 * k;
        if (p.order_mode) { HIP_OK(launch_poa_order(p, st), ABPOA_HIP_ELAUNCH); if (stage("row order", k)) return ABPOA_HIP_ELAUNCH; dbg.order_check(k); }
        HIP_OK(launch_poa_prepare(p, st), ABPOA_HIP_ELAUNCH);
        if (stage("prepare", k)) return ABPOA_HIP_ELAUNCH;
        HIP_OK(hipEventRecord(e[0], st), ABPOA_HIP_ELAUNCH);
        if (general) { HIP_OK(launch_dp_general(b, st), ABPOA_HIP_ELAUNCH); HIP_OK(hipEventRecord(e[1], st), ABPOA_HIP_ELAUNCH); }
        else HIP_OK(launch_dp_fast(b, st, e[1]), ABPOA_HIP_ELAUNCH);
        if (stage("dp rows + tail", k)) return ABPOA_HIP_ELAUNCH;
        if (amb) {
            HIP_OK(launch_poa_strand_check(p, st), ABPOA_HIP_ELAUNCH);
            HIP_OK(launch_dp_general(b_rc, st), ABPOA_HIP_ELAUNCH);
            HIP_OK(launch_poa_strand_pick(p, st), ABPOA_HIP_ELAUNCH);
            if (stage("strand retry", k)) return ABPOA_HIP_ELAUNCH;
        }
        dbg.balance_report(k, b, e[0], e[1]);
        HIP_OK(hipEventRecord(e[2], st), ABPOA_HIP_ELAUNCH);
        HIP_OK(launch_poa_fuse(p, st), ABPOA_HIP_ELAUNCH);
        if (stage("fuse", k)) return ABPOA_HIP_ELAUNCH;
        dbg.graph_check(k);
        HIP_OK(hipEventRecord(e[3], st), ABPOA_HIP_ELAUNCH);
    }
    if (want_cons) { HIP_OK(launch_poa_consensus(p, st), ABPOA_HIP_ELAUNCH); if (stage("consensus", max_reads)) return ABPOA_HIP_ELAUNCH; }
    if (want_msa) { HIP_OK(launch_poa_msa_rank(p, st), ABPOA_HIP_ELAUNCH); if (stage("msa rank", max_reads)) return ABPOA_HIP_ELAUNCH; }
    uint8_t *hg = C.graph.host;
    HIP_OK(hipMemcpyAsync(hg, dg, dl_bytes, hipMemcpyDeviceToHost, st), ABPOA_HIP_ELAUNCH);
    HIP_OK(hipStreamSynchronize(st), ABPOA_HIP_ELAUNCH);
    std::vector<int64_t> msa_off; int64_t msa_total = 0;
    if (want_msa) {
        const PoaState *hs_ = (const PoaState *)(hg + L.o_state);
        msa_off.resize(n_sets);
        for (int s = 0; s < n_sets; ++s) { msa_off[s] = msa_total; if (hs_[s].status == POA_ST_OK && hs_[s].n_nodes > 2) msa_total += (int64_t)(sets[s].n_reads
                + (want_cons ? 1 : 0)) * std::max(0, hs_[s].msa_len); }
        if (msa_total > 0) {
            if ((rc = C.msa.need_dev((size_t)msa_total)) || (rc = C.msa.need_host((size_t)msa_total))) return rc;
            memcpy(hi + L.o_msaoff_h, msa_off.data(), 8 * (size_t)n_sets);
            HIP_OK(hipMemcpyAsync(dg + L.o_msaoff, hi + L.o_msaoff_h, 8 * (size_t)n_sets, hipMemcpyHostToDevice, st), ABPOA_HIP_ELAUNCH);
            p.msa_out = C.msa.dev;
            HIP_OK(launch_poa_msa_fill(p, st), ABPOA_HIP_ELAUNCH);
            if (stage("msa fill", max_reads)) return ABPOA_HIP_ELAUNCH;
            HIP_OK(hipMemcpyAsync(C.msa.host, C.msa.dev, (size_t)msa_total, hipMemcpyDeviceToHost, st), ABPOA_HIP_ELAUNCH);
            HIP_OK(hipStreamSynchronize(st), ABPOA_HIP_ELAUNCH);
        }
    }
    const double t_done = now_s();
    if (opt_env("ABPOA_HIP_ORDER_PROF") && p.order_mode) {
        const PoaState *hs_ = (const PoaState *)(C.graph.host + L.o_state); double a_[4] = {0, 0, 0, 0};
        for (int s = 0; s < n_sets; ++s) for (int i = 0; i < 4; ++i) a_[i] += (double)hs_[s].t_phase[i];
        fprintf(stderr, "[abpoa-hip] order walk per set: %.0f single-node passes x %.0f ticks, %.0f parallel passes x %.0f ticks\n", a_[2] / n_sets,
                a_[2] > 0 ? a_[0] / a_[2] : 0.0, a_[3] / n_sets, a_[3] > 0 ? a_[1] / a_[3] : 0.0);
    }
    if (stats) {
        float ms = 0;
        hipEvent_t prev = C.ev[1];
        for (int k = 1; k < (use_rounds ? 2 : max_reads); ++k) {
            hipEvent_t *e = C.ev.data() + 4 * k;
            (void)hipEventElapsedTime(&ms, prev, e[0]); stats->prepare_ms += ms;
            (void)hipEventElapsedTime(&ms, e[0], e[1]); stats->rows_ms += ms;
            (void)hipEventElapsedTime(&ms, e[1], e[2]); stats->tail_ms += ms;
            (void)hipEventElapsedTime(&ms, e[2], e[3]); stats->fuse_ms += ms;
            prev = e[3];
        }
        if (use_rounds) {
            (void)hipEventElapsedTime(&ms, C.ev[2], C.ev[3]); stats->rounds_ms = ms; stats->rounds_launches = 1;
            const PoaState *hs_ = (const PoaState *)(C.graph.host + L.o_state);
            double tp[4] = {0, 0, 0, 0}, tmax = 0; for (int s = 0; s < n_sets; ++s) { double t_ = 0;
                    if (hs_[s].status == POA_ST_OK) stats->rounds_algo_bytes += hs_[s].algo_bytes - hs_[s].algo_bytes_before;
            for (int i = 0; i < 4; ++i) { tp[i] += (double)hs_[s].t_phase[i]; t_ += (double)hs_[s].t_phase[i]; } tmax = std::max(tmax, t_); }
            const double tall = tp[0] + tp[1] + tp[2] + tp[3];
            if (tall > 0) { stats->prepare_ms += ms * tp[0] / tall; stats->rows_ms += ms * tp[1] / tall; stats->tail_ms += ms * tp[2] / tall;
                    stats->fuse_ms += ms * tp[3] / tall;
                            for (int i = 0; i < 4; ++i) stats->rounds_mticks[i] = tp[i] / n_sets * 1e-6; stats->rounds_rows_share = tp[1] / tall;
                            stats->rounds_mean_over_max = n_sets > 0 && tmax > 0 ? tall / n_sets / tmax : 0; }
        }
        stats->n_rounds = max_reads > 0 ? max_reads - 1 : 0; stats->device_s = t_done - t_queue;
    }

    const PoaState *hs = (const PoaState *)(hg + L.o_state);
    const int32_t *h_cnode = (const int32_t *)(hg + L.o_cnode), *h_ccov = (const int32_t *)(hg + L.o_ccov); const uint8_t *h_cbase = hg + L.o_cbase;
    std::vector<char> need_fb(n_sets, 0);
    parallel_ranges(std::min(n_threads, 8), n_sets, [&](int lo, int hi_) {
        for (int s = lo; s < hi_; ++s) {
            abpoa_hip_msa_t &o_ = out[s];
            memset(&o_, 0, sizeof(o_)); o_.n_reads = sets[s].n_reads;
            if (amb && hs[s].status == POA_ST_OK) { o_.is_rc = (uint8_t *)calloc((size_t)std::max(1, sets[s].n_reads), 1);
                    if (o_.is_rc) memcpy(o_.is_rc, hg + L.o_isrc + ps[s].read0, (size_t)sets[s].n_reads); }
            if (hs[s].status != POA_ST_OK) { need_fb[s] = hs[s].pad == 5 ? 2 : 1;
                    if (dbg_sync) fprintf(stderr, "[poa-device] set %d falls back to the host driver: reason %d, %d nodes of %d\n", s, hs[s].pad,
                    hs[s].n_nodes, ps[s].node_cap); continue; }
            o_.n_cells = hs[s].n_cells;
            if (p.dig_on && sets[s].n_reads > 0) cigar_digest_set(sets[s].seqs[0], sets[s].lens[0], hs[s].cigar_dig);
            if (want_cons && hs[s].n_nodes > 2) {
                const int len = hs[s].cons_len; const int64_t c0 = ps[s].cons0;
                o_.cons_len = len;
                o_.cons_base = (uint8_t *)malloc(len + 1); o_.cons_cov = (int32_t *)malloc(4 * (len + 1)); o_.cons_node_id = (int32_t *)malloc(4 * (len + 1));
                memcpy(o_.cons_base, h_cbase + c0, len); memcpy(o_.cons_cov, h_ccov + c0, 4 * (size_t)len);
                memcpy(o_.cons_node_id, h_cnode + c0, 4 * (size_t)len);
            }
            if (want_msa && hs[s].n_nodes > 2) {
                const int len = std::max(0, hs[s].msa_len);
                o_.msa_len = len; o_.msa_rows = sets[s].n_reads + (want_cons ? 1 : 0);
                o_.msa_base = (uint8_t *)malloc((size_t)o_.msa_rows * (len > 0 ? len : 1));
                if (len > 0) memcpy(o_.msa_base, C.msa.host + msa_off[s], (size_t)o_.msa_rows * len);
            }
        }
    });
    dbg.msa_check(hs, out);
    dbg.consensus_check(hs, out);
    for (int s = 0; s < n_sets; ++s) if (need_fb[s]) fallback->push_back(need_fb[s] == 2 ? -(s + 1) : s);
    if (fallback_reason) {
        fallback_reason->clear();
        for (int s = 0; s < n_sets; ++s) if (need_fb[s]) { const int r = hs[s].pad;
                fallback_reason->push_back(r >= 1000 ? (r - 1000 == ABPOA_HIP_STATUS_OVERFLOW ? 9 : 10) : (r >= 1 && r <= 8 ? r : 0)); }
    }
    if (opt_env("ABPOA_HIP_VERBOSE") && !fallback->empty()) {
        int hist[8] = {0, 0, 0, 0, 0, 0, 0, 0};
        int n_slots = 0;
        int dp_arena = 0, dp_scores = 0, dp_other = 0;
        for (int f : *fallback) {
            const int s = f < 0 ? -f - 1 : f; const int r = hs[s].pad;
            if (r == 5) { n_slots++; continue; }
            if (r >= 1000) { if (r - 1000 == ABPOA_HIP_STATUS_OVERFLOW) dp_arena++; else if (r - 1000 == ABPOA_HIP_STATUS_NEED_SCORES) dp_scores++;
                    else dp_other++; }
            hist[r >= 1000 ? 5 : (r >= 0 && r < 5 ? r : (r == 6 ? 7 : 6))]++;
            if (!(r >= 1000 || (r >= 0 && r < 7))) fprintf(stderr,
                    "[abpoa-hip]   set %d: reason code %d (7: row order walk, 8: MSA rank walk, 1000 + a negative DP status: " "%d)\n", s, r, r - 1000);
        }
        if (hist[5]) fprintf(stderr, "[abpoa-hip]   DP status: arena too small for the bands %d, direction words undecided %d, other %d\n", dp_arena,
                dp_scores, dp_other);
        fprintf(stderr, "[abpoa-hip] fallback reasons: node cap at init %d, pred CSR cap %d, cigar cap %d, node slots in the fuse "
                "phase %d, edge slots of a node full (redone in the last pass) %d, DP status %d, projected node growth "
                "(early exit at read 10) %d, other %d\n", hist[1], hist[2], hist[3], hist[4], n_slots, hist[5], hist[7], hist[6] + hist[0]);
    }
    if (stats) {
        stats->cons_s = now_s() - t_done; stats->total_s = now_s() - t_begin;
        for (int s = 0; s < n_sets; ++s) if (!need_fb[s]) {
            stats->n_cells += hs[s].n_cells; stats->algo_bytes += hs[s].algo_bytes; stats->n_alignments += std::max(0, sets[s].n_reads - 1);
            int mx = 0; for (int r = 0; r < sets[s].n_reads; ++r) mx = std::max(mx, sets[s].lens[r]);
            if ((int64_t)hs[s].n_nodes <= 2 + (int64_t)(3.0 * mx) + 1024) stats->n_fit_3x += 1;
        }
    }
    return ABPOA_HIP_OK;
}


int run_msa_device(const abpoa_hip_scoring_t *sc, int n_sets, const abpoa_hip_readset_t *sets, abpoa_hip_msa_t *out, int n_threads,
                   std::vector<int> *fallback, DeviceRunStats *stats, double node_factor, unsigned flags, int device, int slot, std::vector<int> *fallback_reason) {
    bool want_general = false;
    const int rc = run_msa_device_body(sc, n_sets, sets, out, n_threads, fallback, stats, node_factor, flags, device, slot, false, &want_general, fallback_reason);
    if (rc != ABPOA_HIP_EINVAL || !want_general) return rc;
    want_general = false;
    return run_msa_device_body(sc, n_sets, sets, out, n_threads, fallback, stats, node_factor, flags, device, slot, true, &want_general, fallback_reason);
}

}
```

### abpoa_amd/csrc/poa_rounds.hip

```cpp
#define ABPOA_HIP_ONE_WAVE_PHASE 1
#include "fast_tail.h"
#include "poa_bodies.h"
#include "msa_device.h"

namespace abpoa_hip {

struct RoundsArgs { PoaDev p; DevBatch b; int32_t *cu_ticket; };
__constant__ RoundsArgs g_rounds[MSA_DEVICE_SLOTS];

#define UNI(x) __builtin_amdgcn_readfirstlane(x)
__device__ __noinline__ void rounds_prepare(const int slot, const int s, const int k) { poa_prepare_body(g_rounds[UNI(slot)].p, UNI(s), UNI(k)); }
__device__ __noinline__ void rounds_fuse(const int slot, const int s, const int k) { poa_fuse_body(g_rounds[UNI(slot)].p, UNI(s), UNI(k)); }
__device__ __forceinline__ AlnDesc uniform_desc(const AlnDesc *g) {
    static_assert(sizeof(AlnDesc) % 4 == 0, "AlnDesc is read as 32-bit words");
    AlnDesc d; const int *src = (const int *)g; int *dst = (int *)&d;
#pragma unroll
    for (int i = 0; i < (int)(sizeof(AlnDesc) / 4); ++i) dst[i] = __builtin_amdgcn_readfirstlane(src[i]);
    return d;
}
template <typename T, int GAP, bool DIR>
__device__ __noinline__ long long rounds_rows(const int slot, const int s_) {
    const DevBatch &b = g_rounds[UNI(slot)].b; const int s = UNI(s_);
    const AlnDesc d = uniform_desc(b.aln + s);
    align_fast_rows<T, GAP, 1, false, DIR>(b, d, b.out + s);
    return (long long)__builtin_amdgcn_s_memtime();
}
template <typename T, int GAP, bool DIR>
__device__ __noinline__ void rounds_tail(const int slot, const int s_, const int role_, int *ctl, const int gen_) {
    const DevBatch &b = g_rounds[UNI(slot)].b; const int s = UNI(s_);
    const AlnDesc d = uniform_desc(b.aln + s);
    align_fast_tail<T, GAP, DIR>(b, d, b.out + s, UNI(role_), ctl, UNI(gen_));
}

template <int GAP>
__global__ void __launch_bounds__(GT, 4) poa_rounds_kernel(const int slot, const int k_lo) {
    const int s = blockIdx.x, tid = threadIdx.x;
    const PoaDev &p = g_rounds[slot].p; const DevBatch &b = g_rounds[slot].b;
    if (s >= p.n_sets) return;
    const int n_reads = p.sets[s].n_reads;
    PoaState *st = p.state + s;
    long long t_prep = 0, t_rows = 0, t_tail = 0, t_fuse = 0;
    __shared__ int sh_simd[GW], sh_target, sh_walk[8 * SPEC_WK];
    if (tid < 8 * SPEC_WK) sh_walk[tid] = 0;
    {
        const unsigned hwid = __builtin_amdgcn_s_getreg(63492);
        if ((tid & 63) == 0) sh_simd[tid >> 6] = (int)((hwid >> 4) & 3);
        if (tid == 0) { const unsigned xcc = __builtin_amdgcn_s_getreg(6164) & 15; sh_target = atomicAdd(g_rounds[slot].cu_ticket + ((xcc << 8) | ((hwid >> 8) & 0xff)), 1) & 3; }
        __syncthreads();
    }
    if (tid == 0) st->algo_bytes_before = st->algo_bytes;
    int worker = 0;
#pragma unroll
    for (int w_ = GW - 1; w_ >= 0; --w_) if (sh_simd[w_] == sh_target) worker = w_;
    static_assert(GW == SPEC_WK, "one wavefront of the workgroup per walk of a backtrack");
    const bool pair = !(b.dbg & 1024);
    for (int k = k_lo; k < n_reads; ++k) {
        const long long c0 = (long long)__builtin_amdgcn_s_memtime();
        rounds_prepare(slot, s, k);
        __syncthreads();
        if (ld_fresh(&st->status) != POA_ST_OK) break;
        const long long c1 = (long long)__builtin_amdgcn_s_memtime();
        long long c2 = c1;
        if ((tid >> 6) == worker) {
            const int bits = b.aln[s].bits, w = b.aln[s].w, flags = b.aln[s].flags;
            if ((flags & ALN_FAST_OK) && !(b.lds.wide_nw >= 1 && w >= b.lds.wide_w_lo && w <= b.lds.wide_w_hi)) {
                bool done_dir = false;
                if constexpr (GAP != 0) if (b.dir_mode) {
                    if (bits == 16) { c2 = rounds_rows<int16_t, GAP, true>(slot, s); rounds_tail<int16_t, GAP, true>(slot, s, pair ? 0 : -1, sh_walk, k); }
                    else { c2 = rounds_rows<int32_t, GAP, true>(slot, s); rounds_tail<int32_t, GAP, true>(slot, s, pair ? 0 : -1, sh_walk, k); }
                    done_dir = true;
                }
                if (done_dir) {}
                else if (bits == 16) { c2 = rounds_rows<int16_t, GAP, false>(slot, s); rounds_tail<int16_t, GAP, false>(slot, s, -1, sh_walk, k); }
                else { c2 = rounds_rows<int32_t, GAP, false>(slot, s); rounds_tail<int32_t, GAP, false>(slot, s, -1, sh_walk, k); }
            } else if ((tid & 63) == 0) b.out[s].status = ABPOA_HIP_EINVAL;
        } else if (GAP != 0 && b.dir_mode && pair) {
            if constexpr (GAP != 0) {
            const int bits = b.aln[s].bits, w = b.aln[s].w, flags = b.aln[s].flags, hr = (((int)(tid >> 6) - worker) & (GW - 1));
            if ((flags & ALN_FAST_OK) && !(b.lds.wide_nw >= 1 && w >= b.lds.wide_w_lo && w <= b.lds.wide_w_hi)) {
                if (bits == 16) rounds_tail<int16_t, GAP, true>(slot, s, hr, sh_walk, k); else rounds_tail<int32_t, GAP, true>(slot, s, hr, sh_walk, k);
            }
            }
        }
        __syncthreads();
        const long long c3 = (long long)__builtin_amdgcn_s_memtime();
        rounds_fuse(slot, s, k);
        __syncthreads();
        t_prep += c1 - c0; t_rows += c2 - c1; t_tail += c3 - c2; t_fuse += (long long)__builtin_amdgcn_s_memtime() - c3;
    }
    if (tid == worker * 64) { st->t_phase[0] += t_prep; st->t_phase[1] += t_rows; st->t_phase[2] += t_tail; st->t_phase[3] += t_fuse; }
}

size_t poa_rounds_args_bytes() { return sizeof(RoundsArgs); }
hipError_t launch_poa_rounds(const PoaDev &p, const DevBatch &b, int32_t *cu_ticket, void *host_args, int slot, int k_lo, size_t lds_bytes, hipStream_t s) {
    if (p.n_sets <= 0) return hipSuccess;
    if (slot < 0 || slot >= MSA_DEVICE_SLOTS) return hipErrorInvalidValue;
    RoundsArgs &a = *(RoundsArgs *)host_args;
    a.p = p; a.b = b; a.cu_ticket = cu_ticket;
    hipError_t e = hipMemsetAsync(cu_ticket, 0, 4 * POA_CU_TICKETS, s);
    if (e != hipSuccess) return e;
    e = hipMemcpyToSymbolAsync(HIP_SYMBOL(g_rounds), &a, sizeof(a), sizeof(RoundsArgs) * (size_t)slot, hipMemcpyHostToDevice, s);
    if (e != hipSuccess) return e;
    if (lds_bytes > 65536) {
        e = hipFuncSetAttribute(b.gap_mode == ABPOA_HIP_LINEAR_GAP ? (const void *)poa_rounds_kernel<0> : (b.gap_mode == ABPOA_HIP_AFFINE_GAP ? (const void *)poa_rounds_kernel<1> : (const void *)poa_rounds_kernel<2>),
                hipFuncAttributeMaxDynamicSharedMemorySize, (int)lds_bytes);
        if (e != hipSuccess) return e;
    }
    if (b.gap_mode == ABPOA_HIP_LINEAR_GAP) hipLaunchKernelGGL(poa_rounds_kernel<0>, dim3(p.n_sets), dim3(GT), lds_bytes, s, slot, k_lo);
    else if (b.gap_mode == ABPOA_HIP_AFFINE_GAP) hipLaunchKernelGGL(poa_rounds_kernel<1>, dim3(p.n_sets), dim3(GT), lds_bytes, s, slot, k_lo);
    else hipLaunchKernelGGL(poa_rounds_kernel<2>, dim3(p.n_sets), dim3(GT), lds_bytes, s, slot, k_lo);
    return hipGetLastError();
}
int poa_rounds_residency(int gap_mode, size_t lds_bytes, int *static_lds) {
    int nb = 0; hipFuncAttributes fa; memset(&fa, 0, sizeof(fa));
    if (gap_mode == ABPOA_HIP_LINEAR_GAP) { (void)hipOccupancyMaxActiveBlocksPerMultiprocessor(&nb, poa_rounds_kernel<0>, GT, lds_bytes);
            (void)hipFuncGetAttributes(&fa, (const void *)poa_rounds_kernel<0>); }
    else if (gap_mode == ABPOA_HIP_AFFINE_GAP) { (void)hipOccupancyMaxActiveBlocksPerMultiprocessor(&nb, poa_rounds_kernel<1>, GT, lds_bytes);
            (void)hipFuncGetAttributes(&fa, (const void *)poa_rounds_kernel<1>); }
    else { (void)hipOccupancyMaxActiveBlocksPerMultiprocessor(&nb, poa_rounds_kernel<2>, GT, lds_bytes); (void)hipFuncGetAttributes(&fa, (const void *)poa_rounds_kernel<2>); }
    if (static_lds) *static_lds = (int)fa.sharedSizeBytes;
    return nb;
}

}
```

### abpoa_amd/csrc/rows_fast.h

```cpp
#pragma once
#include "dp_common.h"
#include "dir_plane.h"
#include "rows_tight_asm.h"
#include "wide_closed_forms.h"

namespace abpoa_hip {

template <typename T, int GAP> struct FastFmt { static constexpr int CW = GAP == 0 ? 2 : (GAP == 1 ? 4 : 8); };
template <typename T, int GAP> struct DirFmt {
    static constexpr int DB = GAP == 1 ? 2 : 4;
    static constexpr int UPV2 = Width<T>::PN * DB / 16;
    __device__ __host__ static constexpr int units(int nv) { return (nv * UPV2 + 1) >> 1; }
};
template <int GAP> __device__ __forceinline__ unsigned dir_word(unsigned kf, unsigned u1, unsigned u2, unsigned d1, unsigned d2) {
    static_assert(DIRA_DF1_SH - DIRA_UE1_SH == 3 && DIRC_UE2_SH - DIRC_UE1_SH == 3 && DIRC_DF2_SH - DIRC_DF1_SH == 3 && DIRC_DF1_SH - DIRC_UE1_SH == 8, "field layout of dir_plane.h");
    if (GAP == 1) return (((d1 << 3) | u1) << DIRA_UE1_SH) | kf;
    return (((((d2 << 3) | d1) << 8) | ((u2 << 3) | u1)) << DIRC_UE1_SH) | kf;
}
template <int GAP> __device__ __forceinline__ unsigned dir_pack(unsigned kM, unsigned kE1, unsigned kE2, unsigned u1, unsigned u2, unsigned d1, unsigned d2) {
    return dir_word<GAP>(GAP == 1 ? (kE1 << DIRA_KE1_SH) | kM : (((kE2 << 4) | kE1) << DIRC_KE1_SH) | kM, u1, u2, d1, d2);
}
__device__ __forceinline__ unsigned umin_(unsigned a, unsigned b) { return a < b ? a : b; }
template <typename T> __device__ __forceinline__ unsigned dir_literal(int Hm1, int Fm1, int F, int oe, int e) {
    return (int)(T)(Hm1 - oe) == F ? (unsigned)DIR_LIT_OPEN : ((int)(T)(Fm1 - e) == F ? (unsigned)DIR_LIT_EXT : (unsigned)DIR_LIT_NEITHER);
}
template <typename T> struct FastIO {
    GLOBAL_AS const uint8_t *row_base, *row_sdist; GLOBAL_AS const int32_t *row_remain, *pred_off, *pred_row;
    GLOBAL_AS int32_t *g_bsn, *g_esn, *row_max_i, *g_left, *g_right; GLOBAL_AS int64_t *g_coff;
    T *planes;
};

template <typename T, int GAP>
__device__ __forceinline__ void slow_f_vectors(int vbase, int end_sn, int max_pre, int nfast, int l, int vvl, T hs, T inf,
                                               T e1, T oe1, T o1, T e2, T oe2, T o2, T &F1, T &F2, T &first, T &first2) {
    constexpr int PN = Width<T>::PN, NV = 64 / PN;
#pragma unroll
    for (int vv = 0; vv < NV; ++vv) {
        const int vg = vbase + vv;
        if (vv >= nfast && vg <= end_sn) {
            int set_num = PN;
            if (vg > max_pre) set_num = (vg == max_pre + 1) ? 2 : 1;
            T prev = (T)row_shr<1>((int)first, (int)hs);
            if (PN == 8) prev = (l == 0) ? first : prev;
            T f = wsub<T>(prev, oe1);
            f = set_f<T>(f, l, set_num, e1, inf);
            const T hlast = (T)__builtin_amdgcn_readlane((int)hs, vv * PN + PN - 1);
            first = tmax<T>(hlast, wadd<T>((T)__builtin_amdgcn_readlane((int)f, vv * PN + PN - 1), o1));
            if (vvl == vv) F1 = f;
            if (GAP == 2) {
                T prev2 = (T)row_shr<1>((int)first2, (int)hs);
                if (PN == 8) prev2 = (l == 0) ? first2 : prev2;
                T g = wsub<T>(prev2, oe2);
                g = set_f<T>(g, l, set_num, e2, inf);
                first2 = tmax<T>(hlast, wadd<T>((T)__builtin_amdgcn_readlane((int)g, vv * PN + PN - 1), o2));
                if (vvl == vv) F2 = g;
            }
        }
    }
}

#ifdef ABPOA_HIP_PROFILE
#define FSTAMP(I) { asm volatile("s_waitcnt lgkmcnt(0)" ::: "memory"); long long t_ = (long long)__builtin_amdgcn_s_memtime(); fseg[I] += t_ - fseg_last; fseg_last = t_; }
#else
#define FSTAMP(I)
#endif
#ifdef ABPOA_HIP_ASM_CENSUS
#define CENSUS_SLOT(I) ((I) == 0 ? 1 : (I))
#else
#define CENSUS_SLOT(I) (I)
#endif
#ifdef ABPOA_HIP_ROW_CENSUS
#define CENSUS_T0() const long long cen_t0 = (long long)__builtin_amdgcn_s_memtime();
#define CENSUS(I) { fseg[CENSUS_SLOT(I)] += (1ll << 40) + ((long long)__builtin_amdgcn_s_memtime() - cen_t0); }
#else
#define CENSUS_T0()
#define CENSUS(I)
#endif
#ifdef ABPOA_HIP_WIDE_COUNTERS
#define WCOUNT(I) { fseg[I] += 1; }
#define WCOUNT_BODY(NCH) { fseg[0] += 1 + ((NCH) >= 9 ? (I16 ? 1ll << 48 : 1ll << 32) : 0); }
#else
#define WCOUNT(I) {}
#define WCOUNT_BODY(NCH) {}
#endif
#ifdef ABPOA_HIP_ABLATE
#define ABL(BIT) (b.dbg & (BIT))
#else
#define ABL(BIT) false
#endif
template <typename T, int GAP, int NW = 1, bool WIDEB = false, bool DIR = false, bool XL = false>
__device__ __forceinline__ void rows_fast(const DevBatch &b, const AlnDesc &d, const FastIO<T> &io, const uint8_t *s_query,
                                          long long &cursor_out, long long &n_cells_out, int &status, int &rows_done_out, int &last_done, long long *fseg, int *best_out = nullptr) {
#ifdef ABPOA_HIP_PROFILE
    long long fseg_last = 0;
#endif
    constexpr int PN = Width<T>::PN, NV = 64 / PN;
    constexpr int CW = FastFmt<T, GAP>::CW;
    constexpr bool I16 = sizeof(T) == 2;
    constexpr bool CSP = DIR && WIDEB;
    constexpr int CWR = CSP ? (I16 ? (GAP == 2 ? 4 : 2) : 2) : CW;
    constexpr bool CPK = CSP && !I16 && GAP == 2;
    static_assert(!(DIR && NW > 1), "teams of wavefronts keep the score-record arenas");
    static_assert(!(GAP == 0 && (DIR || NW > 1 || WIDEB)), "linear gaps: the narrow loop with H records only");
    constexpr int DB = DirFmt<T, GAP>::DB, CAPF1 = GAP == 1 ? DIRA_CAP1 : DIRC_CAP1, CAPF2 = DIRC_CAP2;
    auto dir_units = [](int nv) __attribute__((always_inline)) { return DirFmt<T, GAP>::units(nv); };
    auto row_units = [&](int nv, bool spill) __attribute__((always_inline)) { return DIR ? dir_units(nv) + (spill ? nv * CWR : 0) : nv * CW; };
    bool row_spill = false;
    constexpr bool WPLAN = NW > 1 || WIDEB;
    constexpr bool EPACK = WPLAN && !I16 && GAP == 2;
    constexpr int NPW = I16 ? (GAP == 2 ? 2 : 1) : (GAP == 2 ? (EPACK ? 2 : 3) : (GAP == 0 ? 1 : 2));
    constexpr int PL_E1 = 1, PL_E2 = 2, PL_F1 = GAP == 1 ? 2 : 3, PL_F2 = 4;
    constexpr int GEO_RING = 1 << 24;
    const int lane = threadIdx.x & 63, l = lane % PN, vvl = lane / PN;
    const int wid = NW > 1 ? __builtin_amdgcn_readfirstlane((int)(threadIdx.x >> 6)) : 0;
    const int tid = NW > 1 ? (int)threadIdx.x : lane;
    constexpr int NT = NW * 64;
    const int gn = d.n_rows, qlen = d.qlen, m = b.m, m1 = b.m + 1, w = d.w;
    const int inf = d.inf_min;
    const int e1 = b.e1, o1 = b.o1, oe1 = b.o1 + b.e1, e2 = b.e2, o2 = b.o2, oe2 = b.o2 + b.e2;
    const int RR = WPLAN ? b.lds.wfr_rows : b.lds.fr_rows, RC = WIDEB ? (XL ? WIDE_RING_COLS_XL : WIDE_RING_COLS) : (WPLAN ? b.lds.wfr_cols : b.lds.fr_cols), RCS = RC + 4;
    const int ph_off = WPLAN ? b.lds.w_phase_off : b.lds.phase_off;
    int *fr = (int *)(lds_raw + ph_off + b.lds.fr_off);
    int4 *xch = (int4 *)(lds_raw + ph_off + b.lds.wx_off);
    int *bcast = (int *)(xch + 16);
    typedef __attribute__((address_space(3))) int lds_int_t;
    const int vslot = (int)(unsigned)(size_t)(lds_int_t *)fr + 4 * ((threadIdx.x & 63 & (RR - 1)) * (NPW * RCS) + 2);
    auto ring_at = [&](int slot_addr, int col_idx) __attribute__((always_inline)) { return (const int *)(lds_int_t *)(size_t)(unsigned)(slot_addr + 4 * col_idx); };
    int *s_mx = (int *)(lds_raw + (WPLAN ? b.lds.w_mx_off : b.lds.mx_off));
    auto qat = [&](int j) __attribute__((always_inline)) -> int {
        if constexpr (WPLAN) return ((int)s_query[j >> 1] >> ((j & 1) * 4)) & 15; else return (int)s_query[j];
    };
    const int infw = I16 ? (int)(((unsigned)inf & 0xffffu) | ((unsigned)inf << 16)) : inf;
    const int qlen_sn = qlen / PN;
    auto wr = [](int x) __attribute__((always_inline)) { return (int)(T)x; };

    const int idist = inj_dist<PN>(l);
    const int inj1 = idist >= 0 ? inf - idist * e1 : INT_MIN, inj2 = idist >= 0 ? inf - idist * e2 : INT_MIN;
    const int le1 = lane * e1, le2 = lane * e2;
    const int cf1 = oe1 - e1 + le1, cf2 = oe2 - e2 + le2;
    const long long lo_ll = (long long)(I16 ? INT16_MIN : INT32_MIN) + imax(oe1, oe2) + (long long)PN * imax(e1, e2);
    const int fast_lo = (int)lo_ll;
    const int kconst = I16 ? argmax_key16_const(PN, l, vvl) : 0;
    const int ktie = argmax_tie32(PN, l, vvl);

    { GLOBAL_AS const int32_t *g_mat = vgpr_ptr(b.mat); for (int i = tid; i < m * m1; i += NT) { const int bb = i / m1, qc = i - bb * m1; s_mx[i] = qc < m ? g_mat[bb * m + qc] : 0; } }
    for (int i = tid; i < RR * NPW * RCS; i += NT) { const int pl = (i / RCS) % NPW; fr[i] = (I16 && pl == 0) ? infw : ((EPACK && pl == 1) ? 0 : inf); }
    if (NW > 1 && tid < 16) xch[tid] = make_int4(INT_MIN, INT_MIN, I16 ? 0 : INT_MIN, 0);
    WG_SYNC();
    auto ring_put = [&](int slot, int x, int H, int E1, int E2) __attribute__((always_inline)) {
        int *q = fr + slot * (NPW * RCS) + 2 + x;
        if (I16) { q[0] = (int)(((unsigned)H & 0xffffu) | ((unsigned)E1 << 16)); if (GAP == 2) q[RCS] = E2; }
        else { q[0] = H; if (GAP != 0) q[RCS] = E1; if (GAP == 2) q[2 * RCS] = E2; }
    };

    const bool extend = sgpr(b.align_mode == ABPOA_HIP_EXTEND_MODE ? 1 : 0) != 0;
    int ex_best = inf, ex_i = 0, ex_j = 0, ex_rem = 0; bool zstop = false;
    const bool asm_tight_on = sgpr(!(b.dbg & 2048) && RC == 128 && b.align_mode != ABPOA_HIP_EXTEND_MODE ? 1 : 0) != 0;
    int cur = 0, n_vec_lane = 0;
    const int cap_pn = (int)(d.plane_cap / PN > 0x7fffffffLL ? 0x7fffffffLL : d.plane_cap / PN);
    const int cap_turbo = cap_pn - (DIR ? dir_units(NV) + NV * CWR : NV * CW);
    const int remain_end = __builtin_amdgcn_readfirstlane(io.row_remain[gn - 1]);
    int vg_geo = 0, vg_mi = 0, vg_off = 0;
    int vg_vm = 0, rowmax = 0;
    {
        const int r = __builtin_amdgcn_readfirstlane(io.row_remain[0]) - remain_end - 1;
        const int dp_end0 = imin(qlen, imax(0, qlen - r) + w);
        const int end_sn0 = dp_end0 / PN, W0 = (end_sn0 + 1) * PN;
        if ((long long)W0 * CWR > d.plane_cap) { status = ABPOA_HIP_STATUS_OVERFLOW; cursor_out = 0; n_cells_out = 0; rows_done_out = 0; return; }
        const bool ring0 = W0 <= RC && !EPACK;
        T *H = io.planes;
        for (int i = tid; i < W0; i += NT) {
            int h, x1 = inf, x2 = inf, f1 = inf, f2 = inf;
            if (GAP == 0) h = wr(-e1 * i);
            else if (GAP == 1) { const int g = wr(-o1 - e1 * i); h = i == 0 ? 0 : g; x1 = i == 0 ? wr(-oe1) : inf; f1 = i == 0 ? inf : g; }
            else {
                const int g1 = wr(-o1 - e1 * i), g2 = wr(-o2 - e2 * i);
                h = i == 0 ? 0 : imax(g1, g2); x1 = i == 0 ? wr(-oe1) : inf; x2 = i == 0 ? wr(-oe2) : inf; f1 = i == 0 ? inf : g1; f2 = i == 0 ? inf : g2;
            }
            T *cellp = H + (long long)i * CWR;
            if constexpr (CPK) { cellp[0] = (T)h; cellp[1] = (T)(i == 0 ? (int)((unsigned)(h - x1) | ((unsigned)(h - x2) << 16)) : -1); }
            else if constexpr (CSP) { cellp[0] = (T)h; cellp[PL_E1] = (T)x1; if (GAP == 2) { cellp[PL_E2] = (T)x2; cellp[3] = (T)0; } }
            else if constexpr (GAP == 0) { cellp[0] = (T)h; cellp[1] = (T)0; }
// ... 809 lines not shown
                    unsigned l1 = dir_literal<T>(Hm1, F1m1, F1[c], oe1, e1), l2 = 0;
                    if (GAP == 2) { const int F2m1 = wave_shr1(pF2, F2[c]); l2 = dir_literal<T>(Hm1, F2m1, F2[c], oe2, e2); }
                    if (vvl >= nfast_ && (c > 0 || lane > 0)) wd |= GAP == 1 ? l1 << DIRA_LF1_SH : (l1 << DIRC_LF1_SH | l2 << DIRC_LF2_SH);
                }
                char *const dp = Drow + c * 64 * DB;
                if (GAP == 1) *(uint16_t *)dp = (uint16_t)wd; else *(uint32_t *)dp = wd;
            }
            if (DIR && !row_spill) {}
            else if (DIR && !in_band) {}
            else if (TEAM ? (c < cnt && in_band) : (c < NCH - 1 || nch == NCH)) {
                T *H = Hrow + c * 64 * CWR;
                if (CSP) {
                    if (I16 && GAP == 1) *(int *)H = he;
                    else if (I16) { int2 rec; rec.x = he; rec.y = E2out & 0xffff; *(int2 *)H = rec; }
                    else if (GAP == 1) { int2 rec; rec.x = Hout; rec.y = E1out; *(int2 *)H = rec; }
                    else { int2 rec; rec.x = Hout; rec.y = (int)((unsigned)(Hout - E1out) | ((unsigned)(Hout - E2out) << 16)); *(int2 *)H = rec; }
                }
                else if (I16 && GAP == 1) { int2 rec; rec.x = he; rec.y = (int)__builtin_amdgcn_perm((unsigned)mflag, (unsigned)F1[c], 0x05040100u); *(int2 *)H = rec; }
                else if (I16) { int4 rec; rec.x = he; rec.y = (int)(((unsigned)E2out & 0xffffu) | ((unsigned)F1[c] << 16)); rec.z = F2[c] & 0xffff; rec.w = mflag; *(int4 *)H = rec; }
                else if (GAP == 1) { int4 rec; rec.x = Hout; rec.y = E1out; rec.z = F1[c]; rec.w = mflag; *(int4 *)H = rec; }
                else { int4 r0, r1; r0.x = Hout; r0.y = E1out; r0.z = E2out; r0.w = F1[c]; r1.x = F2[c]; r1.y = mflag; r1.z = 0; r1.w = 0; ((int4 *)H)[0] = r0; ((int4 *)H)[1] = r1; }
            }
            if (!TEAM || c < cnt) {
                if (I16) { qd[c * 64] = in_band ? he : infw; if (GAP == 2) qd[RCS + c * 64] = in_band ? E2out : inf; }
                else if (EPACK) { qd[c * 64] = in_band ? Hout : inf; qd[RCS + c * 64] = in_band ? (int)((unsigned)(Hout - E1out) | ((unsigned)(Hout - E2out) << 16)) : 0; }
                else { qd[c * 64] = in_band ? Hout : inf; qd[RCS + c * 64] = in_band ? E1out : inf; if (GAP == 2) qd[2 * RCS + c * 64] = in_band ? E2out : inf; }
            }
        }
        if (!TEAM) { for (int c = NCH; c < (RC >> 6); ++c) { qd[c * 64] = infw; if (NPW > 1) qd[RCS + c * 64] = EPACK ? 0 : inf; if (NPW > 2) qd[2 * RCS + c * 64] = inf; } }
        else {
            int *const qrow = (int *)ring_at(__builtin_amdgcn_readlane(vslot, ti) + 4 * lane, 0);
            for (int c = nch; c < (RC >> 6); ++c) if (c % NW == wid) { qrow[c * 64] = infw; if (NPW > 1) qrow[RCS + c * 64] = EPACK ? 0 : inf; if (NPW > 2) qrow[2 * RCS + c * 64] = inf; }
        }
        FSTAMP(4)
        mi = -1;
        if (I16) { rowmax = argmax_value16(kbst); if (rowmax > inf) mi = argmax_index16(kbst, PN, qlen); }
        else { rowmax = argmax_value32(kbst, vfloor); if (rowmax > inf) mi = argmax_index32(kbst, PN, beg_sn, qlen); }
        return 1;
    };

    auto fast_body = [&](auto npc, int row, int ti) __attribute__((always_inline)) -> int {
        constexpr int NPC = decltype(npc)::value;
        int pr[4], pgeo[4];
        pr[0] = __builtin_amdgcn_readlane(tv_p0, ti);
        pgeo[0] = __builtin_amdgcn_readlane(vg_geo, pr[0] & 63);
        int mn_mi = __builtin_amdgcn_readlane(vg_mi, pr[0] & 63), mx_mi = mn_mi, min_pb = pgeo[0] & 0xfff, allring = pgeo[0];
        max_pe = (pgeo[0] >> 12) & 0xfff;
        auto more = [&](int k, int tvp) __attribute__((always_inline)) {
            pr[k] = __builtin_amdgcn_readlane(tvp, ti); pgeo[k] = __builtin_amdgcn_readlane(vg_geo, pr[k] & 63);
            const int mi_ = __builtin_amdgcn_readlane(vg_mi, pr[k] & 63);
            mn_mi = imin(mn_mi, mi_); mx_mi = imax(mx_mi, mi_); min_pb = imin(min_pb, pgeo[k] & 0xfff); max_pe = imax(max_pe, (pgeo[k] >> 12) & 0xfff); allring &= pgeo[k];
        };
        if (NPC >= 2) more(1, tv_p1);
        if (NPC >= 4) { pr[2] = pr[1]; pgeo[2] = pgeo[1]; pr[3] = pr[1]; pgeo[3] = pgeo[1]; if (np > 2) more(2, tv_p2); if (np > 3) more(3, tv_p3); }
        set_band(std::true_type{}, mn_mi, mx_mi, min_pb);
        const int Wr = (end_sn - beg_sn + 1) * PN;
        if (!(allring & GEO_RING) || Wr > RC) return 0;
        FSTAMP(0)
        if (!reserve()) return 2;
        to_ring = true;
        T *H = io.planes + (long long)off_pn * PN;
        const int my_slot = (row & (RR - 1)) * (NPW * RCS);
        const int nch = (Wr + 63) >> 6;
        refresh_qc();
        const int *mrow = s_mx + base * m1;
        int first = 0, first2 = 0;
        for (int c = 0; c < nch; ++c) {
            const int col = beg_sn * PN + c * 64 + lane;
            int qc = c == 0 ? qoff0 : qoff1;
            if (c >= 2) qc = (col >= 1 && col <= qlen) ? qat(col - 1) : m;
            const int q = mrow[qc];
            int Mv = lane, E1v = inf, E2v = inf, kb = 0, kE1 = 1, kE2 = 1;
            if (!ABL(16)) from_ring(0, pr[0], pgeo[0], col, Mv, E1v, E2v, kb, 1, kE1, kE2, q);
            if (NPC >= 2 && !ABL(16)) from_ring(1, pr[1], pgeo[1], col, Mv, E1v, E2v, kb, 2, kE1, kE2, q);
            if (NPC >= 4) { if (np > 2) from_ring(2, pr[2], pgeo[2], col, Mv, E1v, E2v, kb, 3, kE1, kE2, q); if (np > 3) from_ring(3, pr[3], pgeo[3], col, Mv, E1v, E2v, kb, 4, kE1, kE2, q); }
            FSTAMP(1)
            chunk_tail(c, nch, Wr, Mv, E1v, E2v, q, kb, first, first2, H, my_slot, kE1, kE2);
        }
        pad_ring(nch, my_slot);
        return 1;
    };

    auto general_body = [&](int row, int ti) __attribute__((always_inline)) -> int {
        const int ps = __builtin_amdgcn_readlane(tv_ps, ti);
        int mn_mi = gn, mx_mi = -1, min_pb = 4095; max_pe = -1;
        for (int k = 0; k < np; ++k) {
            int g_, mi_, off_; geo_of(__builtin_amdgcn_readfirstlane(gld_i32(io.pred_row + ps + k)), row, g_, mi_, off_);
            mn_mi = imin(mn_mi, mi_); mx_mi = imax(mx_mi, mi_); min_pb = imin(min_pb, g_ & 0xfff); max_pe = imax(max_pe, (g_ >> 12) & 0xfff);
        }
        if (np == 0) min_pb = 0;
        set_band(std::false_type{}, mn_mi, mx_mi, min_pb);
        const int Wr = (end_sn - beg_sn + 1) * PN;
        to_ring = Wr <= RC;
        if (DIR && !to_ring) row_spill = true;
        if (!reserve()) return 2;
        T *H = io.planes + (long long)off_pn * PN;
        const int my_slot = (row & (RR - 1)) * (NPW * RCS);
        const int nch = (Wr + 63) >> 6;
        refresh_qc();
        const int *mrow = s_mx + base * m1;
        int first = 0, first2 = 0;
        asm volatile("s_waitcnt vmcnt(0)" ::: "memory");
        for (int c = 0; c < nch; ++c) {
            const int rel = c * 64 + lane, col = beg_sn * PN + rel;
            const bool in_band = rel < Wr;
            int qc = c == 0 ? qoff0 : qoff1;
            if (c >= 2) qc = (col >= 1 && col <= qlen) ? qat(col - 1) : m;
            const int q = mrow[qc];
            int Mv = inf, E1v = inf, E2v = inf, kb = 0, kE1 = 1, kE2 = 1;
            for (int k = 0; k < np; ++k) {
                int g_, mi_, off_; const int p = __builtin_amdgcn_readfirstlane(gld_i32(io.pred_row + ps + k)); geo_of(p, row, g_, mi_, off_);
                if ((g_ & GEO_RING) && row - p < RR) {
                    if (k == 0) from_ring(0, p, g_, col, Mv, E1v, E2v, kb, 1, kE1, kE2, q); else from_ring(1, p, g_, col, Mv, E1v, E2v, kb, k + 1, kE1, kE2, q);
                } else {
                    const int pb = g_ & 0xfff, pe = (g_ >> 12) & 0xfff, Wp = (pe - pb + 1) * PN;
                    const int x = col - pb * PN;
                    const bool inH = in_band && (unsigned)x < (unsigned)(Wp + PN), inE = in_band && (unsigned)x < (unsigned)Wp;
                    const T *Hp = io.planes + (long long)(uint32_t)(off_ - (DIR ? (pe - pb + 1) * CWR : 0)) * PN;
                    int hval = inf, ev1 = inf, ev2 = inf;
                    if (inH && (unsigned)(x - 1) < (unsigned)Wp) hval = gld_cell((GLOBAL_AS const T *)(Hp + (long long)(x - 1) * CWR));
                    if constexpr (GAP == 0) {
                        int vert = inf; if (inH && (unsigned)x < (unsigned)Wp) vert = gld_cell((GLOBAL_AS const T *)(Hp + (long long)x * CWR));
                        const int t = imax(wr(hval + q), wr(vert - e1));
                        Mv = k == 0 ? (inH ? t : inf) : (inH ? imax(Mv, t) : Mv);
                        continue;
                    }
                    if constexpr (CPK) { if (inE) { const int h0 = gld_cell((GLOBAL_AS const T *)(Hp + (long long)x * CWR));
                            const unsigned dd = (unsigned)gld_cell((GLOBAL_AS const T *)(Hp + (long long)x * CWR + 1));
                                                    ev1 = (dd & 0xffffu) == 0xffffu ? inf : h0 - (int)(dd & 0xffffu); ev2 = (dd >> 16) == 0xffffu ? inf : h0 - (int)(dd >> 16); } }
                    else
                    if (inE) { ev1 = gld_cell((GLOBAL_AS const T *)(Hp + (long long)x * CWR + PL_E1)); if (GAP == 2) ev2 = gld_cell((GLOBAL_AS const T *)(Hp + (long long)x * CWR + PL_E2)); }
                    if (k == 0) { Mv = hval; E1v = ev1; E2v = ev2; kb = 1; kE1 = 1; kE2 = 1; }
                    else { kb = (inH && hval > Mv) ? k + 1 : kb; if (DIR) { kE1 = (inE && ev1 > E1v) ? k + 1 : kE1; if (GAP == 2) kE2 = (inE && ev2 > E2v) ? k + 1 : kE2; }
                           Mv = inH ? imax(Mv, hval) : Mv; E1v = inE ? imax(E1v, ev1) : E1v; if (GAP == 2) E2v = inE ? imax(E2v, ev2) : E2v; }
                }
            }
            chunk_tail(c, nch, Wr, Mv, E1v, E2v, q, kb, first, first2, H, my_slot, kE1, kE2);
        }
        if (to_ring) pad_ring(nch, my_slot);
        return 1;
    };

#ifdef ABPOA_HIP_PROFILE
    fseg_last = (long long)__builtin_amdgcn_s_memtime();
#endif
    for (int t0 = 0; t0 < gn - 1 && status == 0 && !zstop; t0 += 64) {
#ifdef ABPOA_HIP_ROW_CENSUS
        const long long cen_ts = (long long)__builtin_amdgcn_s_memtime();
#endif
        if (t0 > 0) {
            const int rb = t0 - 64 + lane; if (wid == 0) { io.g_bsn[rb] = vg_geo & 0xfff; io.g_esn[rb] = (vg_geo >> 12) & 0xfff; io.g_coff[rb] = (long long)(uint32_t)vg_off * PN;
                    io.row_max_i[rb] = vg_mi; }
            if (rb >= 1) n_vec_lane += ((vg_geo >> 12) & 0xfff) - (vg_geo & 0xfff) + 1;
        }
        switch_tile(t0);
#ifdef ABPOA_HIP_ROW_CENSUS
        { asm volatile("" :: "v"(tv_meta), "v"(tv_p0), "v"(tv_tb), "v"(tv_rterm)); fseg[4] += (1ll << 40) + ((long long)__builtin_amdgcn_s_memtime() - cen_ts); }
#endif
        const int r_hi = imin(t0 + 64, gn - 1);
        auto commit_row = [&](int ti, bool ring) __attribute__((always_inline)) {
            const int geo_new = sgpr(beg_sn | (end_sn << 12) | (ring ? GEO_RING : 0)), off_new = sgpr(off_pn); mi = sgpr(mi);
            if (__builtin_expect(extend, 0)) {
                const int mx = sgpr(rowmax > inf ? rowmax : inf), rem_row = qlen - rterm + remain_end + 1;
                if (mx > ex_best) { ex_best = mx; ex_i = t0 + ti; ex_j = mi; ex_rem = rem_row; }
                else if (b.zdrop > 0) { int dd = (ex_rem - rem_row) - (mi - ex_j); if (dd < 0) dd = -dd; if (ex_best - mx > b.zdrop + e1 * dd) zstop = true; }
            }
            if constexpr (WPLAN || !I16) {
                const int vm_new = sgpr(rowmax);
                asm volatile("s_mov_b32 m0, %8\n\ts_nop 3\n\tv_writelane_b32 %0, %4, m0\n\tv_writelane_b32 %1, %5, m0\n\tv_writelane_b32 %2, %6, m0\n\tv_writelane_b32 %3, %7, m0"
                             : "+v"(vg_geo), "+v"(vg_mi), "+v"(vg_off), "+v"(vg_vm) : "s"(geo_new), "s"(mi), "s"(off_new), "s"(vm_new), "s"(ti) : "m0");
            } else
            asm volatile("s_mov_b32 m0, %6\n\ts_nop 3\n\tv_writelane_b32 %0, %3, m0\n\tv_writelane_b32 %1, %4, m0\n\tv_writelane_b32 %2, %5, m0"
                         : "+v"(vg_geo), "+v"(vg_mi), "+v"(vg_off) : "s"(geo_new), "s"(mi), "s"(off_new), "s"(ti) : "m0");
        };
        int row = imax(t0, 1);
        while (row < r_hi && !zstop) {
            if constexpr (NW > 1) {
                const int ti = row & 63;
                last_done = row;
                const int meta = __builtin_amdgcn_readlane(tv_meta, ti);
                rterm = __builtin_amdgcn_readlane(tv_rterm, ti);
                base = meta & 0xff; np = (meta >> 8) & 0xff;
                int rc = 0;
                if ((meta >> 19) & 1) {
                    const int nch_ = ilp_band(row, ti);
                    if (nch_ == -2) { status = ABPOA_HIP_STATUS_OVERFLOW; break; }
                    if (nch_ >= 2) rc = ilp_chunks(std::integral_constant<int, (NCHX + NW - 1) / NW>{}, nch_, row, ti);
                    if (rc != 1) WCOUNT(5);
                } else WCOUNT(1);
                if (rc == 1) { WCOUNT(0); commit_row(ti, true); lds_barrier(); ++row; continue; }
                rc = 0;
                asm volatile("s_waitcnt vmcnt(0)" ::: "memory");
                lds_barrier();
                if (wid == 0) {
                    am_key = 0; am_val = INT_MIN; am_v = 0; am_isend = 0; am_any = false;
                    rc = general_body(row, ti);
                    mi = -1;
                    if (rc == 1) {
                        if (I16) {
                            argmax_decode16(wave_max_u32_s(am_key), PN, qlen, inf, rowmax, mi);
                        } else {
                            const int vmax = wave_max_i32_s(am_any ? am_val : INT_MIN);
                            rowmax = vmax;
                            if (vmax > inf) {
                                unsigned key = 0;
                                if (am_any && am_val == vmax) key = ((unsigned)(PN - 1 - l) << 27) | ((unsigned)am_isend << 26) | (0x3FFFFFFu - (unsigned)am_v);
                                const unsigned kb = wave_max_u32_s(key);
                                mi = (int)(0x3FFFFFFu - (kb & 0x3FFFFFFu)) * PN + (PN - 1 - (int)(kb >> 27));
                                if (mi > qlen) mi = -1;
                            }
                        }
                    }
                    if (lane == 0) { bcast[0] = rc; bcast[1] = beg_sn; bcast[2] = end_sn; bcast[3] = off_pn; bcast[4] = mi; bcast[5] = to_ring ? 1 : 0; bcast[6] = cur; bcast[7] = rowmax; }
                }
                lds_barrier();
                rc = __builtin_amdgcn_readfirstlane(bcast[0]); beg_sn = __builtin_amdgcn_readfirstlane(bcast[1]); end_sn = __builtin_amdgcn_readfirstlane(bcast[2]);
                off_pn = __builtin_amdgcn_readfirstlane(bcast[3]); mi = __builtin_amdgcn_readfirstlane(bcast[4]); to_ring = __builtin_amdgcn_readfirstlane(bcast[5]) != 0;
                cur = __builtin_amdgcn_readfirstlane(bcast[6]); rowmax = __builtin_amdgcn_readfirstlane(bcast[7]);
                if (rc == 2) { status = ABPOA_HIP_STATUS_OVERFLOW; break; }
                commit_row(ti, to_ring);
                lds_barrier();
                ++row;
                continue;
            }
            int ok_ = 1;
            if constexpr (!WPLAN && GAP != 0) if (__builtin_expect(two_chunk_streak, 0)) {
                const int ti_ = row & 63, meta_ = __builtin_amdgcn_readlane(tv_meta, ti_);
                if constexpr (DIR) row_spill = (meta_ >> 21) & 1;
                if ((meta_ >> 19) & 1) {
                    CENSUS_T0()
                    last_done = row;
                    rterm = __builtin_amdgcn_readlane(tv_rterm, ti_); base = meta_ & 0xff; np = (meta_ >> 8) & 0xff;
                    const int nch_ = ilp_band(row, ti_);
                    if (nch_ == -2) { status = ABPOA_HIP_STATUS_OVERFLOW; break; }
                    if (nch_ == 2 && ilp_chunks(std::integral_constant<int, 2>{}, nch_, row, ti_) == 1) { commit_row(ti_, true); CENSUS(3) ++row; continue; }
                }
                two_chunk_streak = 0;
            }
            bool cxx_tight = true;
#if !defined(ABPOA_HIP_ABLATE) && !defined(ABPOA_HIP_PROFILE) && (!defined(ABPOA_HIP_ROW_CENSUS) || defined(ABPOA_HIP_ASM_CENSUS)) && !defined(ABPOA_HIP_NO_ASM_TIGHT)
            if constexpr (!WPLAN && I16 && GAP == 1 && DIR) {
                if (asm_tight_on && cur + NV * (r_hi - row) <= cap_turbo) {
                    int code, sM, sTB, sRT, sR2, sP0, sM0, sG0, sSL0, sA, sB, sESN, sBSN, sPB0, sPE0, sNV1, sC0, sP1, sM1, sG1, sSL1, sPB1, sPE1, sP2, sSL2, sPB2, sPE2, sP3, sSL3, sPB3, sPE3;
                    long long inb, amok, msk;
#ifdef ABPOA_HIP_ASM_CENSUS
                    const int asm_row0 = row; const long long asm_t0 = (long long)__builtin_amdgcn_s_memtime();
#endif
                    int infw_v = infw, inf_v = inf; asm("" : "+v"(infw_v), "+v"(inf_v));
                    const int mxb = (int)(unsigned)(size_t)(lds_int_t *)s_mx, qb = (int)(unsigned)(size_t)(lds_int_t *)(const void *)s_query;
                    asm volatile(TIGHT_ASM_I16_AFFINE_DIR
                        : [row] "+s"(row), [cur] "+s"(cur), [qcb] "+s"(qc_beg_sn), [code] "=&s"(code), [geo] "+v"(vg_geo), [mi] "+v"(vg_mi), [off] "+v"(vg_off), [qoff0] "+v"(qoff0),
                          [qoff1] "+v"(qoff1), [sM] "=&s"(sM), [sTB] "=&s"(sTB), [sRT] "=&s"(sRT), [sR2] "=&s"(sR2), [sP0] "=&s"(sP0), [sM0] "=&s"(sM0), [sG0] "=&s"(sG0), [sSL0] "=&s"(sSL0), [sA] "=&s"(sA),
                          [sB] "=&s"(sB), [sESN] "=&s"(sESN), [sBSN] "=&s"(sBSN), [sPB0] "=&s"(sPB0), [sPE0] "=&s"(sPE0), [sNV1] "=&s"(sNV1), [sC0] "=&s"(sC0), [sP1] "=&s"(sP1),
                          [sM1] "=&s"(sM1), [sG1] "=&s"(sG1), [sSL1] "=&s"(sSL1), [sPB1] "=&s"(sPB1), [sPE1] "=&s"(sPE1), [sP2] "=&s"(sP2), [sSL2] "=&s"(sSL2), [sPB2] "=&s"(sPB2),
                          [sPE2] "=&s"(sPE2), [sP3] "=&s"(sP3), [sSL3] "=&s"(sSL3), [sPB3] "=&s"(sPB3), [sPE3] "=&s"(sPE3), [inb] "=&s"(inb), [amok] "=&s"(amok), [msk] "=&s"(msk)
                        : [lane] "v"(lane), [tvmeta] "v"(tv_meta), [tvtb] "v"(tv_tb), [tvr1] "v"(tv_r1), [tvr2] "v"(tv_r2), [tvp2] "v"(tv_p2), [tvp3] "v"(tv_p3), [vslot] "v"(vslot), [le1] "v"(le1), [cf1] "v"(cf1), [inj1] "v"(inj1), [kN] "v"(kN),
                          [kE] "v"(kE), [vvl] "v"(vvl), [vl] "v"(l), [infwv] "v"(infw_v), [infv] "v"(inf_v), [c1] "s"(1 - w), [c2] "s"(1 + w), [qlen] "s"(qlen), [rc] "s"(RC), [mxb] "s"(mxb), [fastlo] "s"(fast_lo),
                          [e1] "s"(e1), [oe1] "s"(oe1), [infk] "s"((int)((((unsigned)(inf + 32768)) << 16) | 0xffffu)), [planes] "s"(io.planes), [rhi] "s"(r_hi), [qb] "s"(qb), [m] "s"(m), [perm] "s"(0x05040100)
                        : "v92", "v93", "v94", "v95", "v96", "v97", "v98", "v99", "v100", "v101", "v102", "v103", "v104", "v105", "v106", "v107", "v108", "v109", "v110", "v111", "v112", "v113", "v114", "v115", "v116", "v117", "v118", "v119",
                          "v120", "v121", "v122", "v123", "v124", "v125", "v126", "v127", "vcc", "scc", "m0", "memory");
                    ok_ = code == 1 ? 0 : (code == 2 ? -1 : 1);
                    cxx_tight = false;
#ifdef ABPOA_HIP_ASM_CENSUS
                    fseg[0] += ((long long)(row - asm_row0) << 40) + ((long long)__builtin_amdgcn_s_memtime() - asm_t0);
#endif
                }
            }
#endif
            if constexpr (!WPLAN) if (cxx_tight) for (;;) {
                const int ti_ = row & 63;
                const int meta_ = __builtin_amdgcn_readlane(tv_meta, ti_);
                if (!__builtin_expect((meta_ >> 17) & 1, 1)) break;
                if constexpr (DIR) row_spill = (meta_ >> 21) & 1;
                CENSUS_T0()
                rterm = __builtin_amdgcn_readlane(tv_rterm, ti_);
                base = meta_ & 0xff; np = (meta_ >> 8) & 0xff;
                ok_ = np == 1 ? turbo_body(std::integral_constant<int, 1>{}, std::false_type{}, row, ti_) : turbo_body(std::integral_constant<int, 2>{}, std::false_type{}, row, ti_);
                if (__builtin_expect(ok_ != 1, 0)) break;
                commit_row(ti_, true);
                CENSUS(np == 1 ? 0 : 1)
                if (++row >= r_hi || zstop) break;
            }
            last_done = row - 1;
            if (row >= r_hi || zstop) break;
            const int ti = row & 63;
            last_done = row;
            CENSUS_T0()
            const int meta = __builtin_amdgcn_readlane(tv_meta, ti);
            rterm = __builtin_amdgcn_readlane(tv_rterm, ti);
            base = meta & 0xff; np = (meta >> 8) & 0xff;
            if constexpr (DIR) row_spill = (meta >> 21) & 1;
            if (!WPLAN && ((meta >> 18) & 1)) {
                if (turbo_body(std::integral_constant<int, 4>{}, std::true_type{}, row, ti) == 1) { commit_row(ti, true); CENSUS(2) ++row; continue; }
            }
            if (!WPLAN && ((meta >> 20) & 1)) {
                if (turbo_body(std::integral_constant<int, 8>{}, std::true_type{}, row, ti) == 1) { commit_row(ti, true); CENSUS(2) ++row; continue; }
            }
            if (!WPLAN && (((meta >> 17) & 1) ? ok_ == 0 : (DIR && ((meta >> 22) & 1)))) {
                const int ok3 = np == 1 ? turbo_body(std::integral_constant<int, 1>{}, std::true_type{}, row, ti) : turbo_body(std::integral_constant<int, 2>{}, std::true_type{}, row, ti);
                if (ok3 == 1) { commit_row(ti, true); CENSUS(np == 1 ? 0 : 1) ++row; continue; }
            }
            if (GAP != 0 && !WPLAN && ((meta >> 19) & 1)) {
                const int nch_ = ilp_band(row, ti);
                if (nch_ == -2) { status = ABPOA_HIP_STATUS_OVERFLOW; break; }
                if (nch_ >= 1 && nch_ <= 2 && ilp_chunks(std::integral_constant<int, 2>{}, nch_, row, ti) == 1) { two_chunk_streak = nch_ == 2; commit_row(ti, true); CENSUS(3) ++row; continue; }
            }
            if (WIDEB && ((meta >> 19) & 1)) {
                const int nch_ = ilp_band(row, ti);
                if (nch_ == -2) { status = ABPOA_HIP_STATUS_OVERFLOW; break; }
                if (nch_ >= 2) {
                    int ok2;
                    if (nch_ <= 3) ok2 = ilp_chunks(std::integral_constant<int, 3>{}, nch_, row, ti);
#ifndef ABPOA_HIP_WIDE_PAIRED_NCH
                    else if (nch_ == 4) ok2 = ilp_chunks(std::integral_constant<int, 4>{}, nch_, row, ti);
                    else if (nch_ == 5) ok2 = ilp_chunks(std::integral_constant<int, 5>{}, nch_, row, ti);
                    else if (nch_ == 6) ok2 = ilp_chunks(std::integral_constant<int, 6>{}, nch_, row, ti);
#else
                    else if (nch_ <= 5) ok2 = ilp_chunks(std::integral_constant<int, 5>{}, nch_, row, ti);
#endif
                    else if (nch_ <= 7) ok2 = ilp_chunks(std::integral_constant<int, 7>{}, nch_, row, ti);
                    else if constexpr (XL) {
                        if (nch_ == 8) ok2 = ilp_chunks(std::integral_constant<int, 8>{}, nch_, row, ti);
                        else if (nch_ == 9) ok2 = ilp_chunks(std::integral_constant<int, 9>{}, nch_, row, ti);
                        else ok2 = ilp_chunks(std::integral_constant<int, 11>{}, nch_, row, ti);
                    }
                    else ok2 = 0;
                    if (ok2 == 1) { WCOUNT_BODY(nch_); commit_row(ti, true); FSTAMP(5) ++row; continue; }
                    WCOUNT(5);
                }
            } else if (WIDEB) WCOUNT(1);
            am_key = 0; am_val = INT_MIN; am_v = 0; am_isend = 0; am_any = false;
            int rc = 0;
            {
                if (!WPLAN && ((meta >> 16) & 1)) {
                    if (np == 1) rc = fast_body(std::integral_constant<int, 1>{}, row, ti);
                    else if (np == 2) rc = fast_body(std::integral_constant<int, 2>{}, row, ti);
                    else rc = fast_body(std::integral_constant<int, 4>{}, row, ti);
                }
                if (rc == 0) rc = general_body(row, ti);
                if (rc == 2) { status = ABPOA_HIP_STATUS_OVERFLOW; break; }
                FSTAMP(3)
                mi = -1;
                if (I16) {
                    argmax_decode16(wave_max_u32_s(am_key), PN, qlen, inf, rowmax, mi);
                } else {
                    const int vmax = wave_max_i32_s(am_any ? am_val : INT_MIN);
                    rowmax = vmax;
                    if (vmax > inf) {
                        unsigned key = 0;
                        if (am_any && am_val == vmax) key = ((unsigned)(PN - 1 - l) << 27) | ((unsigned)am_isend << 26) | (0x3FFFFFFu - (unsigned)am_v);
                        const unsigned kb = wave_max_u32_s(key);
                        mi = (int)(0x3FFFFFFu - (kb & 0x3FFFFFFu)) * PN + (PN - 1 - (int)(kb >> 27));
                        if (mi > qlen) mi = -1;
                    }
                }
            }
            commit_row(ti, to_ring);
            FSTAMP(4)
            CENSUS(3)
#ifdef ABPOA_HIP_ROW_CENSUS
            fseg[5] += np > 4 ? (1ll << 40) : (((meta >> 16) & 1) ? (1ll << 20) : 1ll);
#endif
            ++row;
        }
        if (status != 0) break;
    }
    if (status == 0) {
        const int tb = last_done & ~63, rb = tb + lane;
        if (rb <= last_done) { if (wid == 0) { io.g_bsn[rb] = vg_geo & 0xfff; io.g_esn[rb] = (vg_geo >> 12) & 0xfff; io.g_coff[rb] = (long long)(uint32_t)vg_off * PN; io.row_max_i[rb] = vg_mi; }
                               if (rb >= 1) n_vec_lane += ((vg_geo >> 12) & 0xfff) - (vg_geo & 0xfff) + 1; }
    }
    WG_SYNC();
    if (status == 0 && b.want_lr && wid == 0) {
        const int push_lim = zstop ? last_done : gn;
        for (int r = lane; r < gn; r += 64) {
            int lf = gn, rt = 0;
            if (r == 0) { lf = 0; rt = 0; }
            else for (int k = io.pred_off[r]; k < io.pred_off[r + 1]; ++k) {
                const int p = io.pred_row[k];
                if (p >= push_lim) continue;
                const int oi = (p == 0 ? 0 : io.row_max_i[p]) + 1;
                lf = imin(lf, oi); rt = imax(rt, oi);
            }
            io.g_left[r] = lf; io.g_right[r] = rt;
        }
    }
    if (best_out) { best_out[0] = ex_best; best_out[1] = ex_i; best_out[2] = ex_j; }
    cursor_out = (long long)cur * PN; n_cells_out = (long long)__builtin_amdgcn_readlane(wave_scan_add_i32(n_vec_lane), 63) * PN; rows_done_out = last_done;
}

template <typename T, int GAP, int NW = 1, bool WIDEB = false, bool DIR = false, bool XL = false>
__device__ __forceinline__ void align_fast_rows(const DevBatch &b, const AlnDesc &d, AlnOut *out_rec) {
    const int lane = threadIdx.x & 63;
    FastIO<T> io;
    io.row_base = vgpr_ptr(b.row_base + d.row0); io.row_remain = vgpr_ptr(b.row_remain + d.row0); io.row_sdist = vgpr_ptr((DIR ? b.row_sdist : b.row_base) + d.row0);
    io.pred_off = vgpr_ptr(b.pred_off + d.poff0); io.pred_row = vgpr_ptr(b.pred_row + d.pred0);
    io.g_bsn = vgpr_ptr(b.dp_beg_sn + d.row0); io.g_esn = vgpr_ptr(b.dp_end_sn + d.row0); io.row_max_i = vgpr_ptr(b.row_max_i + d.row0);
    io.g_left = vgpr_ptr(b.left + d.row0); io.g_right = vgpr_ptr(b.right + d.row0); io.g_coff = vgpr_ptr(b.row_cell_off + d.row0);
    io.planes = (T *)(b.planes + d.plane_off);
    uint8_t *s_query = lds_raw + b.lds.q_off;
    { GLOBAL_AS const uint8_t *g_query = vgpr_ptr(b.query + d.query_off);
      if constexpr (NW > 1 || WIDEB) {
          for (int i = (NW > 1 ? (int)threadIdx.x : lane); 2 * i < d.qlen; i += NW * 64) { const int lo_ = g_query[2 * i], hi_ = 2 * i + 1 < d.qlen ? (int)g_query[2 * i + 1] : 0;
                  s_query[i] = (uint8_t)((lo_ & 15) | (hi_ << 4)); }
      } else for (int i = (NW > 1 ? (int)threadIdx.x : lane); i < d.qlen; i += NW * 64) s_query[i] = g_query[i]; }
    WG_SYNC();
    long long cursor = 0, n_cells = 0; int status = 0, rows_done = 0, last_done = 0;
    const long long clk0 = (long long)__builtin_amdgcn_s_memtime();
    long long fseg[6] = {0, 0, 0, 0, 0, 0};
    int best3[3] = {d.inf_min, 0, 0};
    rows_fast<T, GAP, NW, WIDEB, DIR, XL>(b, d, io, s_query, cursor, n_cells, status, rows_done, last_done, fseg, best3);
    const long long clk1 = (long long)__builtin_amdgcn_s_memtime();
#if !defined(ABPOA_HIP_WIDE_COUNTERS) && !defined(ABPOA_HIP_ROW_CENSUS)
    fseg[5] = (long long)__builtin_amdgcn_s_getreg(63492) | ((long long)__builtin_amdgcn_s_getreg(6164) << 32);
#endif
    if (NW > 1 ? threadIdx.x == 0 : lane == 0) { GLOBAL_AS AlnOut *o = vgpr_ptr(out_rec); o->status = status; o->n_cells = n_cells; o->cells_used = cursor; o->clk_dp = clk1 - clk0;
            o->n_rows_done = rows_done; for (int i_ = 0; i_ < 6; ++i_) o->seg[i_] = fseg[i_];
            if (b.align_mode == ABPOA_HIP_EXTEND_MODE) { o->best_score = best3[0]; o->best_row = best3[1]; o->best_col = best3[2]; } }
}


}
```

Before: 18410.

## Start speculative backtrack helper waves under the row loop via LDS progress flag

Helper waves for the paired direction-word backtrack no longer wait for the row loop to finish. They poll an LDS progress counter that the row-loop wave publishes after each tile, and begin walking from their start rows once those rows are complete. To make this possible, LDS is repartitioned into a main region that holds the row ring plus three helper regions, and helper start rows are moved earlier in the graph. The aim is to overlap backtrack with DP. The costs are a vmcnt wait on every tile, polling and sleep overhead, and smaller helper windows. An env option restores the late start, and an arena-size override and verbose per-phase stats are also added.

```diff
diff --git a/abpoa_amd/csrc/backtrack_dir.h b/abpoa_amd/csrc/backtrack_dir.h
--- a/abpoa_amd/csrc/backtrack_dir.h
+++ b/abpoa_amd/csrc/backtrack_dir.h
@@ -12,12 +12,22 @@
 template <int R> struct __attribute__((aligned(16))) DirBtT { int2 rec[R]; int2 pd[R]; int32_t stg[R], rowA[R]; };
 typedef DirBtT<DBTR> DirBt;
 
-constexpr int SPEC_PM_ROWS = 256;
-constexpr int SPEC_WK = 4;
 __device__ __forceinline__ bool dir_walk_pair(const DevBatch &b, const AlnDesc &d) { return d.n_rows >= 768 && d.cigar_cap < 65536 && d.qlen < 65536 && b.ret_cigar; }
+constexpr int SPEC_PROG_FINAL = 1 << 30, SPEC_PROG_ABANDON = -1;
+constexpr int SPEC_WAIT_POLLS = 1 << 16;
+__device__ __forceinline__ bool dir_walk_early(const DevBatch &b, const AlnDesc &d) { return b.lds.te_on != 0 && dir_walk_pair(b, d); }
+__device__ __forceinline__ int spec_start_row(const bool early, const int gn, const int r) {
+    return early ? (int)(((long long)gn * (r == 1 ? 14 : (r == 2 ? 11 : 6))) >> 4) : (int)(((long long)gn * (SPEC_WK - r)) / SPEC_WK);
+}
+__device__ __forceinline__ int spec_region(const DevBatch &b, const bool early, const int r, int &bytes, int &pm_off) {
+    if (early) { bytes = r == 0 ? b.lds.te_main : b.lds.te_w; pm_off = b.lds.te_main + (SPEC_WK - 1) * b.lds.te_w; return r == 0 ? 0 : b.lds.te_main + (r - 1) * b.lds.te_w; }
+    const int total_lds = b.lds.bt_off + b.lds.bt_bytes_tail;
+    bytes = ((total_lds - (SPEC_WK - 1) * SPEC_PM_ROWS * 4) / SPEC_WK) & ~15; pm_off = SPEC_WK * bytes;
+    return r * bytes;
+}
 template <typename T, int GAP, int DBR = DBTR>
 __device__ __forceinline__ void finish_alignment_dir(const DevBatch &b, const AlnDesc &d, AlnOut *out_rec, const TailState &ts, const int role = -1,
-                                                     int *spec_ctl = nullptr, const int gen = 0) {
+                                                     int *spec_ctl = nullptr, const int gen = 0, const int *spec_prog = nullptr) {
     constexpr int PN = Width<T>::PN, CW = FastFmt<T, GAP>::CW, DB = DirFmt<T, GAP>::DB, S = (int)sizeof(T);
     constexpr int ALIGN = 16 / DB;
     constexpr int DBL = DB == 2 ? 1 : 2;
@@ -44,16 +54,28 @@
     WG_SYNC();
     typedef __attribute__((address_space(3))) volatile int lds_vint_t;
     const bool spec_static = role >= 0 && dir_walk_pair(b, d), spec = spec_static && status == 0;
-    auto start_row = [&](int r_) __attribute__((always_inline)) { return (int)(((long long)gn * (SPEC_WK - r_)) / SPEC_WK); };
+    const bool early = spec_static && dir_walk_early(b, d);
+    auto start_row = [&](int r_) __attribute__((always_inline)) { return spec_start_row(early, gn, r_); };
     const int R_g = spec && role >= 1 ? start_row(role) : 0, R_lo = R_g - SPEC_PM_ROWS + 1;
-    const int total_lds = b.lds.bt_off + b.lds.bt_bytes_tail;
-    const int half_lds = spec_static ? ((total_lds - (SPEC_WK - 1) * SPEC_PM_ROWS * 4) / SPEC_WK) & ~15 : total_lds;
-    int *pm_all = (int *)(lds_raw + b.lds.phase_off + SPEC_WK * half_lds);
+    int half_lds = b.lds.bt_off + b.lds.bt_bytes_tail, pm_off = 0, reg_off = 0;
+    if (spec_static) reg_off = spec_region(b, early, role, half_lds, pm_off);
+    int *pm_all = (int *)(lds_raw + b.lds.phase_off + pm_off);
     int *pm = pm_all + (role >= 1 ? role - 1 : 0) * SPEC_PM_ROWS;
     lds_vint_t *ctl = (lds_vint_t *)spec_ctl, *my = ctl + 8 * (role > 0 ? role : 0);
     auto helper_out = [&](int st_) __attribute__((always_inline)) { if (lane == 0) my[1] = st_; asm volatile("s_waitcnt lgkmcnt(0)" ::: "memory"); if (lane == 0) my[0] = gen; };
     if (role >= 1) {
         if (!spec) { if (spec_static) helper_out(-1); return; }
+        if (early) {
+            bool go = false;
+            for (int polls = 0; polls < SPEC_WAIT_POLLS; ++polls) {
+                const int v = ((lds_vint_t *)spec_prog)[0];
+                if (v < 0) break;
+                if ((v & (SPEC_PROG_FINAL - 1)) > R_g) { go = true; break; }
+                if (v & SPEC_PROG_FINAL) break;
+                __builtin_amdgcn_s_sleep(127); __builtin_amdgcn_s_sleep(127);
+            }
+            if (!go) { helper_out(-1); return; }
+        }
         const int c_g = __builtin_amdgcn_readfirstlane(gld_i32(vgpr_ptr(b.row_max_i + d.row0) + R_g));
         if (c_g < 1 || c_g > qlen) { helper_out(-1); return; }
         best_i = R_g; best_j = c_g;
@@ -82,7 +104,7 @@
     int n_cigar = 0, node_s = 0, node_e = 0, query_s = 0, query_e = 0, n_aln = 0, n_match = 0;
     long long win_ticks = 0, walk_ticks = 0; int n_windows = 0, n_general = 0;
     long long dbg_why = 0, dbg_a = 0, dbg_b = 0;
-    if (spec_static && role == 0) {
+    if (spec_static && role == 0 && !early) {
         for (int t = lane; t < (SPEC_WK - 1) * SPEC_PM_ROWS; t += 64) pm_all[t] = 0;
         asm volatile("s_waitcnt lgkmcnt(0)" ::: "memory");
         if (lane == 0) ctl[0] = gen;
@@ -90,7 +112,7 @@
     if (status == 0 && b.ret_cigar && d.cigar_cap < gn + qlen + 2) status = ABPOA_HIP_EBACKTRACK;
     if (role >= 1 && status != 0) { helper_out(-1); return; }
     if (status == 0 && b.ret_cigar) {
-        const int lds0 = b.lds.phase_off + (role >= 1 ? role * half_lds : 0);
+        const int lds0 = b.lds.phase_off + reg_off;
         DirBt &B = *(DirBt *)(lds_raw + lds0);
         unsigned char *win = lds_raw + lds0 + (int)sizeof(DirBt);
         const int win_bytes = half_lds - (int)sizeof(DirBt);
diff --git a/abpoa_amd/csrc/engine.cpp b/abpoa_amd/csrc/engine.cpp
--- a/abpoa_amd/csrc/engine.cpp
+++ b/abpoa_amd/csrc/engine.cpp
@@ -110,6 +110,7 @@
     if (n_aln > 4 * 256 && L.fr_cols && L.fr_cols <= 128) L.bt_bytes_tail = std::min(L.bt_bytes_tail, 12 * 1024);
     { const char *tb_ = opt_env("ABPOA_HIP_BT_BYTES"); if (tb_ && atoi(tb_) >= 4096 && atoi(tb_) <= 65536) L.bt_bytes_tail = atoi(tb_) & ~15; }
     L.total_rows = L.phase_off + L.fr_off + fr_bytes; L.total_tail = L.phase_off + L.bt_off + L.bt_bytes_tail;
+    L.te_on = L.te_main = L.te_w = 0;
     L.bt_wc = 0; { const char *wc_ = opt_env("ABPOA_HIP_BT_WC"); if (wc_ && atoi(wc_) >= 8 && atoi(wc_) <= 64) L.bt_wc = atoi(wc_) & ~7; }
     L.loc_rows = L.loc_cols = L.total_local = 0;
     if (sc->align_mode == ABPOA_HIP_LOCAL_MODE && sc->wb < 0 && P != 1 && L.q_cap && !(opt_env("ABPOA_HIP_NOFAST") && atoi(opt_env("ABPOA_HIP_NOFAST")))) {
diff --git a/abpoa_amd/csrc/engine.h b/abpoa_amd/csrc/engine.h
--- a/abpoa_amd/csrc/engine.h
+++ b/abpoa_amd/csrc/engine.h
@@ -63,7 +63,11 @@
     int32_t mx_off;
     int32_t total;
     int32_t total_rows, total_tail;
+    int32_t te_on, te_main, te_w;
 };
+constexpr int SPEC_PM_ROWS = 256;
+constexpr int SPEC_WK = 4;
+constexpr int SPEC_EARLY_MIN = 6 * 1024;
 
 struct DevBatch {
     int32_t n;
diff --git a/abpoa_amd/csrc/engine_options.cpp b/abpoa_amd/csrc/engine_options.cpp
--- a/abpoa_amd/csrc/engine_options.cpp
+++ b/abpoa_amd/csrc/engine_options.cpp
@@ -20,6 +20,7 @@
     {"ABPOA_HIP_NO_DEVICE_GENERAL", "T  1: general-kernel jobs on the host driver"},
     {"ABPOA_HIP_DEVICE_GENERAL", "T  1: the general kernel for every device-resident job"},
     {"ABPOA_HIP_LOCKSTEP", "T  1: one launch per phase and round also where the all-rounds kernel would run"},
+    {"ABPOA_HIP_LATE_TAIL", "T  1: the helpers of the all-rounds kernel's backtrack start after the row loop, not under it"},
     {"ABPOA_HIP_NODIR", "T  1: score-record arenas instead of direction words"},
     {"ABPOA_HIP_DIR_WIDE", "T  1 / 0: direction words for wide-band alignments always / never (default: by residency and memory)"},
     {"ABPOA_HIP_NOFAST", "T  1: no fast row loops (general kernel)"},
diff --git a/abpoa_amd/csrc/fast_tail.h b/abpoa_amd/csrc/fast_tail.h
--- a/abpoa_amd/csrc/fast_tail.h
+++ b/abpoa_amd/csrc/fast_tail.h
@@ -7,12 +7,15 @@
 namespace abpoa_hip {
 
 template <typename T, int GAP, bool DIR = false>
-__device__ __forceinline__ void align_fast_tail(const DevBatch &b, const AlnDesc &d, AlnOut *out_rec, const int role = -1, int *spec_ctl = nullptr, const int gen = 0) {
+__device__ __forceinline__ void align_fast_tail(const DevBatch &b, const AlnDesc &d, AlnOut *out_rec, const int role = -1, int *spec_ctl = nullptr, const int gen = 0,
+                                                const int *spec_prog = nullptr) {
     const int lane = threadIdx.x & 63;
+    bool early_h = false;
     if (role >= 1) {
         if (!(DIR && takes_dir(b, d) && dir_walk_pair(b, d))) return;
+        if constexpr (DIR) early_h = dir_walk_early(b, d);
         typedef __attribute__((address_space(3))) volatile int lds_vint_t;
-        while (((lds_vint_t *)spec_ctl)[0] != gen) __builtin_amdgcn_s_sleep(4);
+        if (!early_h) while (((lds_vint_t *)spec_ctl)[0] != gen) __builtin_amdgcn_s_sleep(4);
     }
     uint8_t *s_query = lds_raw + b.lds.q_off;
     int32_t *s_mat = (int32_t *)(lds_raw + b.lds.mat_off);
@@ -20,7 +23,7 @@
     if (!dir_a) { GLOBAL_AS const int32_t *g_mat = vgpr_ptr(b.mat); for (int i = lane; i < b.m * b.m; i += 64) s_mat[i] = g_mat[i]; }
     if (!dir_a) { GLOBAL_AS const uint8_t *g_query = vgpr_ptr(b.query + d.query_off); for (int i = lane; i < d.qlen; i += 64) s_query[i] = g_query[i]; }
     TailState ts;
-    ts.status = out_rec->status; ts.n_cells = out_rec->n_cells; ts.cursor = out_rec->cells_used; ts.rows_done = out_rec->n_rows_done;
+    ts.status = early_h ? 0 : out_rec->status; ts.n_cells = out_rec->n_cells; ts.cursor = out_rec->cells_used; ts.rows_done = out_rec->n_rows_done;
     ts.best_score = d.inf_min; ts.best_i = 0; ts.best_j = 0;
     if (b.align_mode == ABPOA_HIP_LOCAL_MODE || b.align_mode == ABPOA_HIP_EXTEND_MODE) { ts.best_score = out_rec->best_score; ts.best_i = out_rec->best_row; ts.best_j = out_rec->best_col; }
     for (int i_ = 0; i_ < 6; ++i_) ts.seg[i_] = out_rec->seg[i_];
@@ -28,7 +31,7 @@
     WG_SYNC();
     if constexpr (DIR) {
         if (!takes_dir(b, d)) finish_alignment<T, GAP, FastFmt<T, GAP>::CW>(b, d, out_rec, ts);
-        else if (role >= 0 && dir_walk_pair(b, d)) finish_alignment_dir<T, GAP, 64>(b, d, out_rec, ts, role, spec_ctl, gen);
+        else if (role >= 0 && dir_walk_pair(b, d)) finish_alignment_dir<T, GAP, 64>(b, d, out_rec, ts, role, spec_ctl, gen, spec_prog);
         else if (role <= 0) finish_alignment_dir<T, GAP>(b, d, out_rec, ts);
     }
     else finish_alignment<T, GAP, FastFmt<T, GAP>::CW>(b, d, out_rec, ts);
diff --git a/abpoa_amd/csrc/msa_device.cpp b/abpoa_amd/csrc/msa_device.cpp
--- a/abpoa_amd/csrc/msa_device.cpp
+++ b/abpoa_amd/csrc/msa_device.cpp
@@ -258,9 +258,12 @@
             const bool dir_s = dir && (dw || !wide_s);
             const int64_t rec_div = (wide_s && wide_ring_rows <= 4) ? 2 : 4;
             const int64_t recb = wide_s ? ((bits == 16 && CW == 4) ? 4 : 8) : CW * (bits / 8);
-            const int64_t bytes = local ? (int64_t)up((size_t)((width * cap + 64) * CW * (bits / 8) + 64 * 8 * 4))
+            int64_t bytes = local ? (int64_t)up((size_t)((width * cap + 64) * CW * (bits / 8) + 64 * 8 * 4))
                                 : dir_s ? (int64_t)up((size_t)(width * (DB + recb) + (est * DB + est * recb / rec_div + 32) * (cap - 1) + 64 * 8 * 4))
                                       : (int64_t)up((size_t)((width + est * (cap - 1)) * CW * (bits / 8) + 64 * 8 * 4));
+            { const char *pct_ = opt_env("ABPOA_HIP_ARENA_PCT");
+              if (pct_ && !local && node_factor <= 3.0 && atoi(pct_) > 0 && atoi(pct_) < 100)
+                  bytes = std::max<int64_t>((int64_t)up((size_t)(2 * width * (DB + recb) + 64 * 8 * 4)), (int64_t)up((size_t)(bytes * atoi(pct_) / 100))); }
             S.plane_off = plane_tot; S.plane_cap = bytes - 64 * 8 * 4; plane_tot += bytes;
         }
     };
@@ -467,12 +470,20 @@
                 rounds_lds = dyn_of(b_r); nb = poa_rounds_residency(sc->gap_mode, rounds_lds, &st_lds);
             }
         }
+        b_r.lds.te_on = 0;
+        if (b_r.dir_mode && sc->gap_mode != ABPOA_HIP_LINEAR_GAP && !(opt_env("ABPOA_HIP_LATE_TAIL") && atoi(opt_env("ABPOA_HIP_LATE_TAIL")))) {
+            const int avail = (int)rounds_lds - b_r.lds.phase_off, tables = (SPEC_WK - 1) * SPEC_PM_ROWS * 4;
+            const int ring = (b_r.lds.total_rows - b_r.lds.phase_off + 15) & ~15;
+            int w_ = ((avail - tables) / SPEC_WK) & ~15, m_ = w_;
+            if (w_ < ring) { m_ = ring; w_ = ((avail - tables - m_) / (SPEC_WK - 1)) & ~15; }
+            if (w_ >= SPEC_EARLY_MIN) { b_r.lds.te_on = 1; b_r.lds.te_main = m_; b_r.lds.te_w = w_; }
+        }
         int n_cu = 256; { hipDeviceProp_t pr; if (hipGetDeviceProperties(&pr, device) == hipSuccess && pr.multiProcessorCount > 0) n_cu =
                 pr.multiProcessorCount; }
         if (nb < 1 || n_sets > nb * n_cu) use_rounds = false;
         if (opt_env("ABPOA_HIP_VERBOSE")) fprintf(stderr,
-                "[abpoa-hip] all-rounds kernel: %s, %zu B dynamic + %d B static LDS per workgroup, %d workgroups per CU, " "backtrack window %d B\n",
-                use_rounds ? "on" : "off", rounds_lds, st_lds, nb, b_r.lds.bt_bytes_tail);
+                "[abpoa-hip] all-rounds kernel: %s, %zu B dynamic + %d B static LDS per workgroup, %d workgroups per CU, " "backtrack window %d B, helpers %s (%d + 3 x %d B)\n",
+                use_rounds ? "on" : "off", rounds_lds, st_lds, nb, b_r.lds.bt_bytes_tail, b_r.lds.te_on ? "under the row loop" : "after the row loop", b_r.lds.te_main, b_r.lds.te_w);
     }
 
     DeviceDebug dbg(&p, &ps, sets, n_sets, sc->m, aln_cap, max_reads, want_msa, amb, st);
@@ -572,6 +583,18 @@
                     stats->fuse_ms += ms * tp[3] / tall;
                             for (int i = 0; i < 4; ++i) stats->rounds_mticks[i] = tp[i] / n_sets * 1e-6; stats->rounds_rows_share = tp[1] / tall;
                             stats->rounds_mean_over_max = n_sets > 0 && tmax > 0 ? tall / n_sets / tmax : 0; }
+            if (opt_env("ABPOA_HIP_VERBOSE") && n_sets > 0 && tall > 0) {
+                static const char *const ph_[4] = {"prepare", "rows", "backtrack", "fuse"};
+                std::vector<double> v_((size_t)n_sets);
+                for (int i = 0; i < 4; ++i) {
+                    for (int s = 0; s < n_sets; ++s) v_[s] = (double)hs_[s].t_phase[i];
+                    std::sort(v_.begin(), v_.end());
+                    fprintf(stderr, "[abpoa-hip] all-rounds kernel, M ticks per set, %-9s: mean %.3f  p99 %.3f  max %.3f\n", ph_[i], tp[i] / n_sets * 1e-6,
+                            v_[(size_t)std::min<long long>(n_sets - 1, (long long)n_sets * 99 / 100)] * 1e-6, v_[(size_t)n_sets - 1] * 1e-6);
+                }
+                fprintf(stderr, "[abpoa-hip] all-rounds kernel, set totals: mean %.3f M ticks, max %.3f M ticks, max / mean %.3f\n", tall / n_sets * 1e-6, tmax * 1e-6,
+                        tmax / (tall / n_sets));
+            }
         }
         stats->n_rounds = max_reads > 0 ? max_reads - 1 : 0; stats->device_s = t_done - t_queue;
     }
diff --git a/abpoa_amd/csrc/poa_rounds.hip b/abpoa_amd/csrc/poa_rounds.hip
--- a/abpoa_amd/csrc/poa_rounds.hip
+++ b/abpoa_amd/csrc/poa_rounds.hip
@@ -19,17 +19,24 @@
     return d;
 }
 template <typename T, int GAP, bool DIR>
-__device__ __noinline__ long long rounds_rows(const int slot, const int s_) {
+__device__ __noinline__ long long rounds_rows(const int slot, const int s_, int *prog) {
     const DevBatch &b = g_rounds[UNI(slot)].b; const int s = UNI(s_);
     const AlnDesc d = uniform_desc(b.aln + s);
-    align_fast_rows<T, GAP, 1, false, DIR>(b, d, b.out + s);
+    if constexpr (DIR) {
+        if (prog && takes_dir(b, d) && dir_walk_early(b, d)) {
+            int bytes_, pm_off_; (void)spec_region(b, true, 0, bytes_, pm_off_);
+            int *pm_all = (int *)(lds_raw + b.lds.phase_off + pm_off_);
+            for (int t = threadIdx.x & 63; t < (SPEC_WK - 1) * SPEC_PM_ROWS; t += 64) pm_all[t] = 0;
+        } else prog = nullptr;
+        align_fast_rows<T, GAP, 1, false, DIR>(b, d, b.out + s, prog);
+    } else align_fast_rows<T, GAP, 1, false, DIR>(b, d, b.out + s);
     return (long long)__builtin_amdgcn_s_memtime();
 }
 template <typename T, int GAP, bool DIR>
 __device__ __noinline__ void rounds_tail(const int slot, const int s_, const int role_, int *ctl, const int gen_) {
     const DevBatch &b = g_rounds[UNI(slot)].b; const int s = UNI(s_);
     const AlnDesc d = uniform_desc(b.aln + s);
-    align_fast_tail<T, GAP, DIR>(b, d, b.out + s, UNI(role_), ctl, UNI(gen_));
+    align_fast_tail<T, GAP, DIR>(b, d, b.out + s, UNI(role_), ctl, UNI(gen_), ctl + 8 * SPEC_WK);
 }
 
 template <int GAP>
@@ -40,8 +47,8 @@
     const int n_reads = p.sets[s].n_reads;
     PoaState *st = p.state + s;
     long long t_prep = 0, t_rows = 0, t_tail = 0, t_fuse = 0;
-    __shared__ int sh_simd[GW], sh_target, sh_walk[8 * SPEC_WK];
-    if (tid < 8 * SPEC_WK) sh_walk[tid] = 0;
+    __shared__ int sh_simd[GW], sh_target, sh_walk[8 * SPEC_WK + 1];
+    if (tid < 8 * SPEC_WK + 1) sh_walk[tid] = 0;
     {
         const unsigned hwid = __builtin_amdgcn_s_getreg(63492);
         if ((tid & 63) == 0) sh_simd[tid >> 6] = (int)((hwid >> 4) & 3);
@@ -56,6 +63,7 @@
     const bool pair = !(b.dbg & 1024);
     for (int k = k_lo; k < n_reads; ++k) {
         const long long c0 = (long long)__builtin_amdgcn_s_memtime();
+        if (tid == 0) sh_walk[8 * SPEC_WK] = 0;
         rounds_prepare(slot, s, k);
         __syncthreads();
         if (ld_fresh(&st->status) != POA_ST_OK) break;
@@ -66,13 +74,14 @@
             if ((flags & ALN_FAST_OK) && !(b.lds.wide_nw >= 1 && w >= b.lds.wide_w_lo && w <= b.lds.wide_w_hi)) {
                 bool done_dir = false;
                 if constexpr (GAP != 0) if (b.dir_mode) {
-                    if (bits == 16) { c2 = rounds_rows<int16_t, GAP, true>(slot, s); rounds_tail<int16_t, GAP, true>(slot, s, pair ? 0 : -1, sh_walk, k); }
-                    else { c2 = rounds_rows<int32_t, GAP, true>(slot, s); rounds_tail<int32_t, GAP, true>(slot, s, pair ? 0 : -1, sh_walk, k); }
+                    int *prog = pair ? sh_walk + 8 * SPEC_WK : nullptr;
+                    if (bits == 16) { c2 = rounds_rows<int16_t, GAP, true>(slot, s, prog); rounds_tail<int16_t, GAP, true>(slot, s, pair ? 0 : -1, sh_walk, k); }
+                    else { c2 = rounds_rows<int32_t, GAP, true>(slot, s, prog); rounds_tail<int32_t, GAP, true>(slot, s, pair ? 0 : -1, sh_walk, k); }
                     done_dir = true;
                 }
                 if (done_dir) {}
-                else if (bits == 16) { c2 = rounds_rows<int16_t, GAP, false>(slot, s); rounds_tail<int16_t, GAP, false>(slot, s, -1, sh_walk, k); }
-                else { c2 = rounds_rows<int32_t, GAP, false>(slot, s); rounds_tail<int32_t, GAP, false>(slot, s, -1, sh_walk, k); }
+                else if (bits == 16) { c2 = rounds_rows<int16_t, GAP, false>(slot, s, nullptr); rounds_tail<int16_t, GAP, false>(slot, s, -1, sh_walk, k); }
+                else { c2 = rounds_rows<int32_t, GAP, false>(slot, s, nullptr); rounds_tail<int32_t, GAP, false>(slot, s, -1, sh_walk, k); }
             } else if ((tid & 63) == 0) b.out[s].status = ABPOA_HIP_EINVAL;
         } else if (GAP != 0 && b.dir_mode && pair) {
             if constexpr (GAP != 0) {
diff --git a/abpoa_amd/csrc/rows_fast.h b/abpoa_amd/csrc/rows_fast.h
--- a/abpoa_amd/csrc/rows_fast.h
+++ b/abpoa_amd/csrc/rows_fast.h
@@ -28,6 +28,7 @@
     GLOBAL_AS const uint8_t *row_base, *row_sdist; GLOBAL_AS const int32_t *row_remain, *pred_off, *pred_row;
     GLOBAL_AS int32_t *g_bsn, *g_esn, *row_max_i, *g_left, *g_right; GLOBAL_AS int64_t *g_coff;
     T *planes;
+    int prog_a;
 };
 
 template <typename T, int GAP>
@@ -1143,6 +1144,10 @@
             const int rb = t0 - 64 + lane; if (wid == 0) { io.g_bsn[rb] = vg_geo & 0xfff; io.g_esn[rb] = (vg_geo >> 12) & 0xfff; io.g_coff[rb] = (long long)(uint32_t)vg_off * PN;
                     io.row_max_i[rb] = vg_mi; }
             if (rb >= 1) n_vec_lane += ((vg_geo >> 12) & 0xfff) - (vg_geo & 0xfff) + 1;
+            if constexpr (DIR && NW == 1 && !WIDEB) if (io.prog_a >= 0) {
+                asm volatile("s_waitcnt vmcnt(0)" ::: "memory");
+                *(volatile lds_int_t *)(size_t)(unsigned)io.prog_a = t0;
+            }
         }
         switch_tile(t0);
 #ifdef ABPOA_HIP_ROW_CENSUS
@@ -1381,9 +1386,11 @@
 }
 
 template <typename T, int GAP, int NW = 1, bool WIDEB = false, bool DIR = false, bool XL = false>
-__device__ __forceinline__ void align_fast_rows(const DevBatch &b, const AlnDesc &d, AlnOut *out_rec) {
+__device__ __forceinline__ void align_fast_rows(const DevBatch &b, const AlnDesc &d, AlnOut *out_rec, const int *prog = nullptr) {
     const int lane = threadIdx.x & 63;
+    typedef __attribute__((address_space(3))) int lds_int_t;
     FastIO<T> io;
+    io.prog_a = -1; if (prog) { io.prog_a = (int)(unsigned)(size_t)(lds_int_t *)prog; asm("" : "+v"(io.prog_a)); }
     io.row_base = vgpr_ptr(b.row_base + d.row0); io.row_remain = vgpr_ptr(b.row_remain + d.row0); io.row_sdist = vgpr_ptr((DIR ? b.row_sdist : b.row_base) + d.row0);
     io.pred_off = vgpr_ptr(b.pred_off + d.poff0); io.pred_row = vgpr_ptr(b.pred_row + d.pred0);
     io.g_bsn = vgpr_ptr(b.dp_beg_sn + d.row0); io.g_esn = vgpr_ptr(b.dp_end_sn + d.row0); io.row_max_i = vgpr_ptr(b.row_max_i + d.row0);
@@ -1408,6 +1415,10 @@
     if (NW > 1 ? threadIdx.x == 0 : lane == 0) { GLOBAL_AS AlnOut *o = vgpr_ptr(out_rec); o->status = status; o->n_cells = n_cells; o->cells_used = cursor; o->clk_dp = clk1 - clk0;
             o->n_rows_done = rows_done; for (int i_ = 0; i_ < 6; ++i_) o->seg[i_] = fseg[i_];
             if (b.align_mode == ABPOA_HIP_EXTEND_MODE) { o->best_score = best3[0]; o->best_row = best3[1]; o->best_col = best3[2]; } }
+    if (io.prog_a >= 0) {
+        asm volatile("s_waitcnt vmcnt(0)" ::: "memory");
+        *(volatile lds_int_t *)(size_t)(unsigned)io.prog_a = status == 0 ? ((last_done + 1) | (1 << 30)) : -1;
+    }
 }
 
 
```

Measured after the change: 19230, median of 6. 1.04x the previous value.
